# allenai/OLMoASR

Hardware: AMD Instinct MI355X
Metric: audio-seconds/sec/node (train step) (higher is better)
Workload: dtype bf16

## Files before the change

include/oasr_testing.h:

```cpp
#ifndef OASR_TESTING_H
#define OASR_TESTING_H
#include "oasr.h"
#ifdef __cplusplus
extern "C" {
#endif

int oasr_profile_gemm(int enable);
int oasr_gemm_set_variant(int v);
int oasr_decode_set_ln_fold(int mode);
int oasr_span_set_side_streams(int mode);
int oasr_span_side_streams(void);
int oasr_xcd_plan_debug(int d, int H, int Te, int M, int L, int team, int wg, int* out, int max_blocks);
int oasr_wide_supports_debug(int d, int H, int Te, int S_max, int L, int M, int nwg, int V);
int oasr_wide_plan_debug(int d, int nwg, int N, int K, int wg, int wave, int* out, int max_units);
int oasr_xcd_offsets_ok_debug(const int64_t* layer0, long long lstride, long long cache_lstride, int d, int Te, int L, int M);
int oasr_attention_set_pingpong(int on);
int oasr_attention_set_span_grid(int on);
int oasr_gemm_set_stagger(int sleeps, int phases);
int oasr_gemm_force_general(int on);
int oasr_test_gemm(const oasr_gemm_args* a, float* colsum_scratch, int atomic_on_pp, int raster_gm, int stagger, int stagger_phases, void* stream);
int oasr_profile_gemm_records(char* buf, int cap);
int oasr_gemm_route_debug(int M, int N, int K, int ta, int tb, int a_view, int b_view, int split_k, int atomic, int atomic_on_pp, int outputs,
                          int sides, long long ldc, long long ldr, long long ldu, int misalign, int colsum, int colsum_scratch, int forced_path,
                          int pp_schedule, int geom_env, char* symbol, int cap, int* post);
int oasr_profile_gemm_collect(double* ms4, double* flops4, int64_t* count4, char* by_symbol , int cap);
int oasr_probe_lds_oob(const void* src_u16 , void* dst_u16 , void* stream);
int oasr_probe_tr16(const void* src_bf16 , void* dst_bf16 , void* stream);
int oasr_test_span_tables(const int32_t* span_host, int B, int S, const int64_t* targets, int32_t* rows_out, int32_t* span_out,
                          int64_t* targets_rows_out, int64_t* active_rows_out, void* stream);
int oasr_test_span_block_tables(const int32_t* span_host, int B, int S, int H, const int64_t* targets, int32_t* rows_out, int32_t* span_out,
                                int64_t* targets_rows_out, int32_t* blk128_out, int32_t* blk256_out, int32_t* counts_out, void* stream);

int oasr_test_embedding_fwd(const int64_t* tok, const float* E, const float* pos, void* x, int dtype, int B, int S, int d, int64_t n_embed,
                            const int32_t* rows, void* stream);
int oasr_test_embedding_bwd(const int64_t* tok, const void* dx, int dtype, float* dE, float* dpos, int B, int S, int d, int64_t pad_id,
                            int64_t n_embed, const int32_t* rows, const int32_t* span, void* stream);
int oasr_test_colsum(const void* x, int dtype, int64_t ld, int64_t M, int ncols, float* out, void* stream);
int oasr_test_conv2_col2im_dgelu(const void* dA, const void* u1, void* dpre1, int dtype, int B, int T1, int d, void* stream);
int oasr_test_conv1_col2im_mel(const void* dcol, int dtype, float* dmel, int B, int T1, int n_mels, void* stream);
int oasr_test_mel_to_time_major(const float* mel, void* out, int dtype, int B, int n_mels, int T, const float* clip_max, void* stream);
int oasr_test_pack_conv_weight(const float* w, void* dst, int dtype, int co, int ci, int ldk, void* stream);
int oasr_test_unpack_conv_grad(const float* g, float* dw, int co, int ci, int ldk, void* stream);
int oasr_test_pack_embedding(const float* e, void* dst, int rows, int rows_pad, int d, void* stream);
int oasr_test_dgelu_mul(const void* dy, const void* u, void* out, int dtype, int64_t n, void* stream);
int oasr_test_dlogits_from_f32(const float* src, int V, int64_t rows, int64_t ld, void* dst, int dtype, void* stream);
int oasr_test_logits_to_f32(const void* logits, int dtype, int64_t ld, int64_t rows, int V, float* out, void* stream);
int oasr_test_layernorm_bwd(const void* dy, const void* x, const float* gamma, const float* mean, const float* rstd, const void* dres, void* dx,
                            float* dgamma, float* dbeta, float* dsum, int dtype, int64_t rows, int d, void* stream);

int oasr_test_dtw_host(const float* cost, int64_t ld, int N, int M, int negate, int32_t* text_indices, int32_t* time_indices, int32_t* path_len,
                       void* workspace);

int oasr_test_argmax_rows(const void* logits, int dtype, int64_t ld, int V, int64_t n_rows, const int32_t* rows, const int32_t* span, int B, int S,
                          int32_t* pred_out, void* stream);

int oasr_test_cross_entropy(void* logits, int dtype, int64_t ld, int V, const int64_t* targets, int64_t rows, int64_t ignore, float gscale,
                            int32_t* n_valid_dev, float* row_loss, float* loss_out, int write_grad, float label_smoothing, float z_loss,
                            float* row_parts, void* stream);

#ifdef __cplusplus
}
#endif
#endif
```

olmoasr_amd/_native.py:

```python
import ctypes as C
import os

import torch

_HERE = os.path.dirname(os.path.abspath(__file__))
LIB_PATH = os.environ.get("OASR_LIB") or os.path.join(_HERE, "liboasr.so")
_lib = None


class NativeError(RuntimeError):
    pass


class Dims(C.Structure):
    _fields_ = [(n, C.c_int) for n in ("n_mels", "n_audio_ctx", "n_audio_state", "n_audio_head", "n_audio_layer",
                                       "n_vocab", "n_text_ctx", "n_text_state", "n_text_head", "n_text_layer")]


class Operand(C.Structure):
    _fields_ = [("ptr", C.c_void_p), ("ld", C.c_int64), ("rpb", C.c_int), ("bstride", C.c_int64), ("lead", C.c_int),
                ("kvalid", C.c_int), ("trail_from", C.c_int)]


class GemmArgs(C.Structure):
    _fields_ = [("A", Operand), ("B", Operand), ("M", C.c_int), ("N", C.c_int), ("K", C.c_int), ("ta", C.c_int),
                ("tb", C.c_int), ("alpha", C.c_float), ("bias", C.c_void_p), ("act", C.c_int), ("pos", C.c_void_p),
                ("pos_period", C.c_int), ("dgelu_u", C.c_void_p), ("ldu", C.c_int64), ("resid", C.c_void_p),
                ("ldr", C.c_int64), ("out", C.c_void_p), ("out_pre", C.c_void_p), ("ldc", C.c_int64),
                ("out_f32", C.c_void_p), ("ldc32", C.c_int64), ("beta", C.c_float), ("colsum", C.c_void_p), ("atomic", C.c_int),
                ("split_k", C.c_int), ("dgelu_deriv", C.c_int)]


class AttnArgs(C.Structure):
    _fields_ = [("q", C.c_void_p), ("k", C.c_void_p), ("v", C.c_void_p), ("ldq", C.c_int64), ("ldk", C.c_int64),
                ("ldv", C.c_int64), ("bsq", C.c_int64), ("bsk", C.c_int64), ("bsv", C.c_int64), ("o", C.c_void_p),
                ("ldo", C.c_int64), ("bso", C.c_int64), ("lse", C.c_void_p), ("o_lo", C.c_void_p), ("kv_len", C.c_void_p), ("B", C.c_int),
                ("H", C.c_int), ("Tq", C.c_int), ("Tk", C.c_int), ("causal", C.c_int), ("d_o", C.c_void_p),
                ("delta", C.c_void_p), ("dq", C.c_void_p), ("dk", C.c_void_p), ("dv", C.c_void_p), ("dq_colsum", C.c_void_p),
                ("dv_colsum", C.c_void_p), ("colsum_scratch", C.c_void_p), ("qtile_flags", C.c_void_p),
                ("q_rows", C.c_void_p), ("k_rows", C.c_void_p), ("q_span", C.c_void_p),
                ("qblk128", C.c_void_p), ("qblk256", C.c_void_p), ("n128", C.c_int), ("n256", C.c_int)]


class AlignArgs(C.Structure):
    MAX_LAYERS = 32
    _fields_ = [("qk", C.c_void_p * 32), ("head_mask", C.c_uint32 * 32), ("n_layers", C.c_int32), ("H", C.c_int32), ("n_tok", C.c_int32),
                ("Tk", C.c_int32), ("n_frames", C.c_int32), ("medfilt_width", C.c_int32), ("qk_scale", C.c_float), ("reserved", C.c_int32),
                ("out", C.c_void_p), ("ldo", C.c_int64)]


class SpecAug(C.Structure):
    MAX_MASKS = 8
    _fields_ = [("freq_masks", C.c_int32), ("freq_width", C.c_int32), ("time_masks", C.c_int32), ("time_width", C.c_int32), ("fill", C.c_float)]


class EditArgs(C.Structure):
    MAX_LEN = 1023
    _fields_ = [("hyp", C.c_void_p), ("ref", C.c_void_p), ("hyp_len", C.c_void_p), ("ref_len", C.c_void_p), ("out", C.c_void_p),
                ("ld_hyp", C.c_int64), ("ld_ref", C.c_int64), ("B", C.c_int32), ("Lh", C.c_int32), ("Lr", C.c_int32), ("reserved", C.c_int32)]


class ScoreArgs(C.Structure):
    _fields_ = [(n, C.c_void_p) for n in ("mel", "xa", "tokens", "targets", "text_len", "span", "row_nll", "pred", "nll_sum", "nll_max", "n_tok",
                                          "n_hit")] + [("B", C.c_int32), ("S", C.c_int32)]


class BeamArgs(C.Structure):
    MAX_BEAM = 15
    NOT_FULL = 0x7fffffff
    _fields_ = [(n, C.c_void_p) for n in ("top_logprob", "top_token", "tokens_in", "tokens_out", "sums", "sources", "last_token", "pool_tokens",
                                          "pool_len", "pool_score", "pool_count", "pool_full_len", "short_step")] + \
               [(n, C.c_int32) for n in ("n_audio", "beam", "max_candidates", "n_ctx", "len", "reserved")] + [("eot", C.c_int64)]


class Speed(C.Structure):
    MAX_FACTORS = 8
    _fields_ = [("n_factors", C.c_int32), ("P", C.c_int32 * 8), ("Q", C.c_int32 * 8)]


class SpeedArgs(C.Structure):
    MAX_N = 1 << 26
    _fields_ = [("pcm_in", C.c_void_p), ("pcm_out", C.c_void_p), ("n_valid", C.c_void_p), ("n_out", C.c_void_p), ("factor_out", C.c_void_p),
                ("tokens_a", C.c_void_p), ("tokens_b", C.c_void_p), ("ld_in", C.c_int64), ("ld_out", C.c_int64), ("ld_tokens_a", C.c_int64),
                ("ld_tokens_b", C.c_int64), ("seed", C.c_uint64), ("first_clip", C.c_uint64), ("B", C.c_int32), ("N", C.c_int32),
                ("S", C.c_int32), ("ts_begin", C.c_int32), ("ts_max", C.c_int32), ("policy", Speed)]


class Noise(C.Structure):
    NONE = -128
    SNR_MIN, SNR_MAX = -10, 50
    _fields_ = [("prob_q16", C.c_int32), ("snr_lo_db", C.c_int32), ("snr_hi_db", C.c_int32)]


class NoiseArgs(C.Structure):
    MAX_N, MAX_ROWS = 1 << 26, 65535
    _fields_ = [("pcm_in", C.c_void_p), ("pcm_out", C.c_void_p), ("n_valid", C.c_void_p), ("bank", C.c_void_p), ("row_out", C.c_void_p),
                ("snr_out", C.c_void_p), ("gain_out", C.c_void_p), ("workspace", C.c_void_p), ("workspace_bytes", C.c_size_t),
                ("ld_in", C.c_int64), ("ld_out", C.c_int64), ("ld_bank", C.c_int64), ("seed", C.c_uint64), ("first_clip", C.c_uint64),
                ("B", C.c_int32), ("N", C.c_int32), ("M", C.c_int32), ("L", C.c_int32), ("policy", Noise), ("reserved", C.c_int32)]


class Reverb(C.Structure):
    _fields_ = [("prob_q16", C.c_int32)]


class ReverbArgs(C.Structure):
    MAX_N, MAX_ROWS, MAX_K, TAP_MAX = 1 << 26, 65535, 8192, 32639
    _fields_ = [("pcm_in", C.c_void_p), ("pcm_out", C.c_void_p), ("n_valid", C.c_void_p), ("rir", C.c_void_p), ("delay", C.c_void_p),
                ("row_out", C.c_void_p), ("workspace", C.c_void_p), ("workspace_bytes", C.c_size_t), ("ld_in", C.c_int64), ("ld_out", C.c_int64),
                ("ld_rir", C.c_int64), ("seed", C.c_uint64), ("first_clip", C.c_uint64), ("B", C.c_int32), ("N", C.c_int32), ("R", C.c_int32),
                ("K", C.c_int32), ("policy", Reverb), ("reserved", C.c_int32)]


class Telephone(C.Structure):
    MAX_CODECS = 8
    LINEAR, MULAW, ALAW = 0, 1, 2
    BP_TAPS, UP_TAPS = 129, 32
    _fields_ = [("prob_q16", C.c_int32), ("n_codecs", C.c_int32), ("codecs", C.c_int32 * 8), ("bandpass", C.c_int32)]


class TelephoneArgs(C.Structure):
    MAX_N, MAX_ROWS = 1 << 26, 65535
    _fields_ = [("pcm_in", C.c_void_p), ("pcm_out", C.c_void_p), ("n_valid", C.c_void_p), ("codec_out", C.c_void_p), ("ld_in", C.c_int64),
                ("ld_out", C.c_int64), ("seed", C.c_uint64), ("first_clip", C.c_uint64), ("B", C.c_int32), ("N", C.c_int32),
                ("policy", Telephone), ("reserved", C.c_int32)]


class TrainStepArgs(C.Structure):
    _fields_ = [(n, C.c_void_p) for n in ("mel", "xa", "tokens", "targets", "text_len", "span_host", "mel_clip_max", "loss_out", "logits_out",
                                          "pred_out", "seg_events")] + \
               [(n, C.c_int32) for n in ("B", "S", "span_forward", "accumulate_loss")] + [("loss_scale", C.c_float), ("inv_accum", C.c_float)] + \
               [("label_smoothing", C.c_float), ("z_loss", C.c_float), ("loss_parts_out", C.c_void_p), ("loss_parts_rows", C.c_void_p)]


DTW_MAX_N, DTW_MAX_M = 448, 1500
STRUCT_SIZES = [
    ("oasr_sizeof_attn_args", AttnArgs),
    ("oasr_sizeof_align_args", AlignArgs),
    ("oasr_sizeof_specaug", SpecAug),
    ("oasr_sizeof_edit_args", EditArgs),
    ("oasr_sizeof_beam_args", BeamArgs),
    ("oasr_sizeof_speed", Speed),
    ("oasr_sizeof_speed_args", SpeedArgs),
    ("oasr_sizeof_noise", Noise),
    ("oasr_sizeof_noise_args", NoiseArgs),
    ("oasr_sizeof_reverb", Reverb),
    ("oasr_sizeof_reverb_args", ReverbArgs),
    ("oasr_sizeof_telephone", Telephone),
    ("oasr_sizeof_telephone_args", TelephoneArgs),
    ("oasr_sizeof_train_step_args", TrainStepArgs),
    ("oasr_sizeof_score_args", ScoreArgs),
]
ABI_VERSION = 216
KV_TAIL_BYTES = 327680
KV_TEAM_COUNTER, KV_ERROR, KV_TEAM_EPOCH, KV_XCC_MASK, KV_WIDE_EPOCH, KV_CTRL_WORDS = 0, 1, 2, 3, 4, 5
KV_REPLICAS, KV_FLAG_STRIDE, KV_FLAGS_WORD = 8, 1024, 1024
MODE_INFER, MODE_TRAIN, MODE_TRAIN_ENC, MODE_TRAIN_DEC = 0, 1, 2, 3
ROWTAB = 16
LORA_MAX_RANK = 64


def _declare(lib):
    vp, i32, i64, f32, sz = C.c_void_p, C.c_int, C.c_int64, C.c_float, C.c_size_t
    sig = {
        "oasr_last_error": (C.c_char_p, []),
        "oasr_version": (i32, []),
        "oasr_log_mel_workspace_bytes": (sz, [i32]),
        "oasr_log_mel": (i32, [vp, i32, i32, i32, vp, vp, vp]),
        "oasr_mel_filterbank": (i32, [vp]),
        "oasr_create": (vp, [C.POINTER(Dims)]),
        "oasr_create_ex": (vp, [C.POINTER(Dims), i32]),
        "oasr_create_ex2": (vp, [C.POINTER(Dims), i32, i32]),
        "oasr_compute_dtype": (i32, [vp]),
        "oasr_create_ex3": (vp, [C.POINTER(Dims), i32, i32, vp, i32, i32, f32]),
        "oasr_lora_count": (i32, [vp]),
        "oasr_lora_merge": (i32, [vp, vp]),
        "oasr_lora_merge_op": (i32, [vp, vp, vp, i32, i32, i32, f32, i32, vp, vp]),
        "oasr_lora_grad_scratch_bytes": (sz, [i32, i32, i32]),
        "oasr_lora_grad_op": (i32, [vp, vp, vp, i32, i32, i32, f32, vp, vp, vp, vp]),
        "oasr_encode": (i32, [vp, vp, i32, vp, vp, sz, vp]),
        "oasr_kv_cache_bytes": (sz, [vp, i32]),
        "oasr_decode_step_workspace_bytes": (sz, [vp, i32]),
        "oasr_decode_begin": (i32, [vp, vp, i32, vp, vp]),
        "oasr_decode_step": (i32, [vp, vp, i32, i32, vp, vp, vp, sz, vp]),
        "oasr_decode_check": (i32, [vp, i32, vp, vp]),
        "oasr_decode_logits": (i32, [vp, vp, vp, vp, i32, i32, i32, vp, vp, sz, vp]),
        "oasr_destroy": (None, [vp]),
        "oasr_param_count": (i32, [vp]),
        "oasr_param_info": (i32, [vp, i32, C.c_char_p, i32, C.POINTER(i64), C.POINTER(i64), C.POINTER(i32), C.POINTER(i64)]),
        "oasr_param_numel": (i64, [vp]),
        "oasr_segment_count": (i32, [vp]),
        "oasr_segment_info": (i32, [vp, i32, C.POINTER(i64), C.POINTER(i64)]),
        "oasr_bind": (i32, [vp, vp, vp, vp, vp, vp]),
        "oasr_shadow_bytes": (sz, [vp]),
        "oasr_bind_shadow": (i32, [vp, vp]),
        "oasr_refresh_shadow": (i32, [vp, vp]),
        "oasr_workspace_bytes": (sz, [vp, i32, i32, i32]),
        "oasr_forward": (i32, [vp, vp, vp, vp, i32, i32, vp, vp, vp, sz, vp]),
        "oasr_sizeof_train_step_args": (sz, []),
        "oasr_train_step": (i32, [vp, C.POINTER(TrainStepArgs), vp, sz, vp]),
        "oasr_log_mel_raw": (i32, [vp, i32, i32, i32, vp, vp, vp, vp]),
        "oasr_sizeof_attn_args": (sz, []),
        "oasr_test_span_tables": (i32, [vp, i32, i32, vp, vp, vp, vp, vp, vp]),
        "oasr_test_span_block_tables": (i32, [vp, i32, i32, i32, vp, vp, vp, vp, vp, vp, vp, vp]),
        "oasr_test_embedding_fwd": (i32, [vp, vp, vp, vp, i32, i32, i32, i32, i64, vp, vp]),
        "oasr_test_embedding_bwd": (i32, [vp, vp, i32, vp, vp, i32, i32, i32, i64, i64, vp, vp, vp]),
        "oasr_test_colsum": (i32, [vp, i32, i64, i64, i32, vp, vp]),
        "oasr_test_conv2_col2im_dgelu": (i32, [vp, vp, vp, i32, i32, i32, i32, vp]),
        "oasr_test_conv1_col2im_mel": (i32, [vp, i32, vp, i32, i32, i32, vp]),
        "oasr_test_mel_to_time_major": (i32, [vp, vp, i32, i32, i32, i32, vp, vp]),
        "oasr_test_pack_conv_weight": (i32, [vp, vp, i32, i32, i32, i32, vp]),
        "oasr_test_unpack_conv_grad": (i32, [vp, vp, i32, i32, i32, vp]),
        "oasr_test_pack_embedding": (i32, [vp, vp, i32, i32, i32, vp]),
        "oasr_test_dgelu_mul": (i32, [vp, vp, vp, i32, i64, vp]),
        "oasr_test_dlogits_from_f32": (i32, [vp, i32, i64, i64, vp, i32, vp]),
        "oasr_test_logits_to_f32": (i32, [vp, i32, i64, i64, i32, vp, vp]),
        "oasr_test_layernorm_bwd": (i32, [vp, vp, vp, vp, vp, vp, vp, vp, vp, vp, i32, i64, i32, vp]),
        "oasr_train_fwd": (i32, [vp, vp, vp, vp, i32, i32, vp, vp, sz, vp]),
        "oasr_train_bwd": (i32, [vp, vp, vp, vp, i32, i32, vp, vp, sz, vp]),
        "oasr_zero_grad": (i32, [vp, vp]),
        "oasr_train_encode": (i32, [vp, vp, i32, vp, vp, sz, vp]),
        "oasr_train_encode_bwd": (i32, [vp, vp, i32, vp, vp, sz, vp]),
        "oasr_train_decode": (i32, [vp, vp, vp, vp, i32, i32, vp, vp, sz, vp]),
        "oasr_train_decode_bwd": (i32, [vp, vp, vp, vp, i32, i32, vp, vp, sz, vp]),
        "oasr_set_trainable": (i32, [vp, vp, i32]),
        "oasr_optim_step": (i32, [vp, f32, f32, f32, f32, f32, f32, f32, i64, vp, vp, vp]),
        "oasr_grad_sumsq_range": (i32, [vp, i64, i64, vp, vp, vp]),
        "oasr_optim_step_range": (i32, [vp, i64, i64, vp, vp, vp, f32, f32, f32, f32, f32, f32, f32, i64, vp]),
        "oasr_gemm": (i32, [C.POINTER(GemmArgs), vp]),
        "oasr_test_gemm": (i32, [C.POINTER(GemmArgs), vp, i32, i32, i32, i32, vp]),
        "oasr_profile_gemm_records": (i32, [C.c_char_p, i32]),
        "oasr_gemm_route_debug": (i32, [i32] * 11 + [i32, C.c_longlong, C.c_longlong, C.c_longlong] + [i32] * 6 + [C.c_char_p, i32, C.POINTER(i32)]),
        "oasr_layernorm_fwd": (i32, [vp, vp, vp, vp, vp, vp, i64, i32, vp]),
        "oasr_layernorm_bwd": (i32, [vp, vp, vp, vp, vp, vp, vp, vp, vp, i64, i32, vp]),
        "oasr_attention_fwd": (i32, [C.POINTER(AttnArgs), vp]),
        "oasr_attention_bwd": (i32, [C.POINTER(AttnArgs), vp]),
        "oasr_attention_scores": (i32, [C.POINTER(AttnArgs), i32, vp, vp]),
        "oasr_sizeof_align_args": (sz, []),
        "oasr_alignment_workspace_bytes": (sz, [i32, i32, i32]),
        "oasr_alignment_matrix": (i32, [C.POINTER(AlignArgs), vp, sz, vp]),
        "oasr_dtw_workspace_bytes": (sz, [i32, i32]),
        "oasr_dtw": (i32, [vp, i64, i32, i32, i32, vp, vp, vp, vp, sz, vp]),
        "oasr_test_dtw_host": (i32, [vp, i64, i32, i32, i32, vp, vp, vp, vp]),
        "oasr_sizeof_specaug": (sz, []),
        "oasr_spec_augment": (i32, [vp, i32, i32, i32, C.POINTER(SpecAug), C.c_uint64, C.c_uint64, vp]),
        "oasr_spec_augment_plan": (i32, [C.POINTER(SpecAug), C.c_uint64, C.c_uint64, i32, i32, vp, vp]),
        "oasr_sizeof_edit_args": (sz, []),
        "oasr_edit_counts": (i32, [C.POINTER(EditArgs), vp]),
        "oasr_edit_counts_host": (i32, [C.POINTER(EditArgs)]),
        "oasr_sizeof_score_args": (sz, []),
        "oasr_score": (i32, [vp, C.POINTER(ScoreArgs), vp, sz, vp]),
        "oasr_score_rows": (i32, [vp, i32, i64, i32, vp, vp, i32, i32, i64, vp, vp, vp]),
        "oasr_score_reduce": (i32, [vp, vp, vp, vp, i32, i32, i32, i64, vp, vp, vp, vp, vp]),
        "oasr_score_reduce_host": (i32, [vp, vp, vp, vp, i32, i32, i32, i64, vp, vp, vp, vp]),
        "oasr_sizeof_beam_args": (sz, []),
        "oasr_beam_update": (i32, [C.POINTER(BeamArgs), vp]),
        "oasr_beam_update_host": (i32, [C.POINTER(BeamArgs)]),
        "oasr_decode_reorder": (i32, [vp, vp, i32, i32, i32, vp, vp, vp]),
        "oasr_decode_reorder_host": (i32, [vp, i64, i32, i32, i32, i32, i32, i32, i32, vp]),
        "oasr_sizeof_speed": (sz, []),
        "oasr_sizeof_speed_args": (sz, []),
        "oasr_speed_perturb": (i32, [C.POINTER(SpeedArgs), vp]),
        "oasr_speed_perturb_host": (i32, [C.POINTER(SpeedArgs)]),
        "oasr_speed_plan": (i32, [C.POINTER(Speed), C.c_uint64, C.c_uint64, i32, i32, C.POINTER(i32), C.POINTER(i32), C.POINTER(i32), C.POINTER(i32)]),
        "oasr_speed_table": (i32, [i32, i32, vp, C.POINTER(i32)]),
        "oasr_sizeof_noise": (sz, []),
        "oasr_sizeof_noise_args": (sz, []),
        "oasr_noise_workspace_bytes": (sz, [i32, i32]),
        "oasr_noise_mix": (i32, [C.POINTER(NoiseArgs), vp]),
        "oasr_noise_mix_host": (i32, [C.POINTER(NoiseArgs)]),
        "oasr_noise_plan": (i32, [C.POINTER(Noise), C.c_uint64, C.c_uint64, i32, i32, C.POINTER(i32), C.POINTER(i32), C.POINTER(i32), C.POINTER(i32)]),
        "oasr_sizeof_reverb": (sz, []),
        "oasr_sizeof_reverb_args": (sz, []),
        "oasr_reverb_workspace_bytes": (sz, [i32, i32]),
        "oasr_reverb": (i32, [C.POINTER(ReverbArgs), vp]),
        "oasr_reverb_host": (i32, [C.POINTER(ReverbArgs)]),
        "oasr_reverb_plan": (i32, [C.POINTER(Reverb), C.c_uint64, C.c_uint64, i32, C.POINTER(i32), C.POINTER(i32)]),
        "oasr_sizeof_telephone": (sz, []),
        "oasr_sizeof_telephone_args": (sz, []),
        "oasr_telephone": (i32, [C.POINTER(TelephoneArgs), vp]),
        "oasr_telephone_host": (i32, [C.POINTER(TelephoneArgs)]),
        "oasr_telephone_plan": (i32, [C.POINTER(Telephone), C.c_uint64, C.c_uint64, C.POINTER(i32), C.POINTER(i32)]),
        "oasr_telephone_tables": (i32, [vp, vp]),
        "oasr_telephone_quantize_host": (i32, [vp, vp, i64, i32]),
        "oasr_test_argmax_rows": (i32, [vp, i32, i64, i32, i64, vp, vp, i32, i32, vp, vp]),
        "oasr_cross_entropy": (i32, [vp, i64, i32, vp, i64, i64, f32, vp, vp, vp, i32, vp]),
        "oasr_cross_entropy_ex": (i32, [vp, i64, i32, vp, i64, i64, f32, vp, vp, vp, i32, f32, f32, vp, vp]),
        "oasr_test_cross_entropy": (i32, [vp, i32, i64, i32, vp, i64, i64, f32, vp, vp, vp, i32, f32, f32, vp, vp]),
        "oasr_cast_f32_bf16": (i32, [vp, vp, i64, vp]),
        "oasr_pick_tokens": (i32, [vp, i64, i32, i64, vp, vp, vp, vp, vp]),
        "oasr_pick_tokens_ts": (i32, [vp, i64, i32, i64, vp, vp, vp, i64, i32, i32, i32, i32, i32, vp, vp, vp]),
        "oasr_topk_tokens": (i32, [vp, i64, i32, i64, vp, vp, vp, i64, i32, i32, i32, i32, i32, i32, vp, vp, vp]),
        "oasr_sample_tokens": (i32, [vp, i64, i32, i64, vp, vp, vp, i64, i32, i32, i32, i32, i32, f32, vp, vp, vp, vp]),
        "oasr_probe_tr16": (i32, [vp, vp, vp]),
        "oasr_probe_lds_oob": (i32, [vp, vp, vp]),
        "oasr_profile_gemm": (i32, [i32]),
        "oasr_gemm_force_general": (i32, [i32]),
        "oasr_gemm_set_stagger": (i32, [i32, i32]),
        "oasr_gemm_set_variant": (i32, [i32]),
        "oasr_decode_set_ln_fold": (i32, [i32]),
        "oasr_span_set_side_streams": (i32, [i32]),
        "oasr_span_side_streams": (i32, []),
        "oasr_xcd_plan_debug": (i32, [i32, i32, i32, i32, i32, i32, i32, vp, i32]),
        "oasr_xcd_offsets_ok_debug": (i32, [vp, C.c_longlong, C.c_longlong, i32, i32, i32, i32]),
        "oasr_wide_supports_debug": (i32, [i32, i32, i32, i32, i32, i32, i32, i32]),
        "oasr_wide_plan_debug": (i32, [i32, i32, i32, i32, i32, i32, vp, i32]),
        "oasr_attention_set_pingpong": (i32, [i32]),
        "oasr_attention_set_span_grid": (i32, [i32]),
        "oasr_profile_gemm_collect": (i32, [vp, vp, vp, C.c_char_p, i32]),
    }
    for name, (res, args) in sig.items():
        fn = getattr(lib, name)
        fn.restype = res
        fn.argtypes = args
    return list(sig)


EXPORTS = None


def _check_struct_size(handle, entry, struct):
    size = getattr(handle, entry, lambda: None)()
    if size != C.sizeof(struct):
        raise NativeError(f"{LIB_PATH}: {entry} answers {size} bytes, this binding's {struct.__name__} has {C.sizeof(struct)} "
                          "-- rebuild (__graft_entry__.build())")


def lib():
    global _lib, EXPORTS
    if _lib is None:
        if not os.path.isfile(LIB_PATH):
            raise NativeError(f"{LIB_PATH} not found: run `python -c 'import __graft_entry__ as g; g.build()'` "
                              "(hipcc --offload-arch=gfx950).  There is no CPU/PyTorch fallback for this path.")
        try:
            _lib = C.CDLL(LIB_PATH)
        except OSError as e:
            raise NativeError(f"cannot load {LIB_PATH}: {e}") from e
        handle, _lib = _lib, None
        ver = getattr(handle, "oasr_version", lambda: None)()
        if ver != ABI_VERSION:
            raise NativeError(f"{LIB_PATH}: ABI version {ver}, this binding is written for version {ABI_VERSION} -- rebuild (__graft_entry__.build())")
        _check_struct_size(handle, *STRUCT_SIZES[0])
        try:
            exports = _declare(handle)
        except AttributeError as e:
            raise NativeError(f"{LIB_PATH} (ABI {ver}) lacks an entry point this binding declares: {e} -- rebuild (__graft_entry__.build())") from e
        for row in STRUCT_SIZES[1:]:
            _check_struct_size(handle, *row)
        _lib, EXPORTS = handle, exports
    return _lib


def enable_testing_hooks():
    os.environ["OASR_TESTING_HOOKS"] = "1"


ERETRY = -4


def check(rc, what=""):
    if rc != 0:
        msg = lib().oasr_last_error()
        raise NativeError(f"{what} failed (rc={rc}): {msg.decode() if msg else ''}")


def ptr(t):
    if t is None:
        return None
    return C.c_void_p(t.data_ptr())


def stream_ptr(device=None):
    return C.c_void_p(torch.cuda.current_stream(device).cuda_stream)


STREAM = object()
_Tensor = torch.Tensor


def call(name, *args, device=None):
    fn = getattr(_lib or lib(), name)
    argv, stream_at = [], -1
    for a in args:
        if isinstance(a, _Tensor):
            if a.is_cuda:
                if device is None:
                    device = a.device
                elif a.device != device:
                    raise NativeError(f"{name}: arguments on {device} and on {a.device} -- one call, one device (nothing was launched)")
            a = a.data_ptr()
        elif a is STREAM:
            stream_at = len(argv)
        argv.append(a)
    if device is None:
        if stream_at >= 0:
            raise NativeError(f"{name}: a stream was asked for, but no argument names a device")
        rc = fn(*argv)
    else:
        with torch.cuda.device(device):
            if stream_at >= 0:
                argv[stream_at] = torch.cuda.current_stream().cuda_stream
            rc = fn(*argv)
    if rc != 0:
        check(rc, name)


def require_gpu(t, name="tensor"):
    if not (isinstance(t, torch.Tensor) and t.is_cuda):
        raise NativeError(f"{name} must be a CUDA/HIP tensor: the MI355X-native path has no CPU fallback")
```

olmoasr_amd/csrc/api.hip:

```cpp
#include <stdarg.h>

#include "../../include/oasr.h"
#include "kernels.h"

static thread_local char g_err[512] = "";

void oasr_set_error(const char* fmt, ...) {
  va_list ap;
  va_start(ap, fmt);
  vsnprintf(g_err, sizeof(g_err), fmt, ap);
  va_end(ap);
}

extern "C" const char* oasr_last_error(void) { return g_err; }
extern "C" int oasr_version(void) { return OASR_ABI_VERSION; }
extern "C" size_t oasr_sizeof_attn_args(void) { return sizeof(oasr_attn_args); }

static OperandView to_view(const oasr_operand& o) {
  return OperandView{(const bf16_t*)o.ptr, (long)o.ld, o.rpb, (long)o.bstride, o.lead, o.kvalid, o.trail_from};
}

static int to_gemm(const oasr_gemm_args* a, GemmArgs& g) {
  OASR_REQUIRE(a, "oasr_gemm: null args");
  g = gemm_defaults();
  g.A = to_view(a->A);
  g.B = to_view(a->B);
  g.M = a->M;
  g.N = a->N;
  g.K = a->K;
  g.ta = a->ta;
  g.tb = a->tb;
  g.alpha = a->alpha;
  g.bias = a->bias;
  g.act = a->act;
  g.pos = a->pos;
  g.pos_period = a->pos_period;
  g.dgelu_u = (const bf16_t*)a->dgelu_u;
  g.ldu = a->ldu;
  g.resid = (const bf16_t*)a->resid;
  g.ldr = a->ldr;
  g.out = (bf16_t*)a->out;
  g.out_pre = (bf16_t*)a->out_pre;
  g.ldc = a->ldc;
  g.out_f32 = a->out_f32;
  g.ldc32 = a->ldc32;
  g.beta = a->beta;
  g.colsum = a->colsum;
  g.atomic = a->atomic;
  g.split_k = a->split_k < 1 ? 1 : a->split_k;
  g.dgelu_deriv = a->dgelu_deriv;
  OASR_REQUIRE(a->act >= 0 && a->act <= 2, "oasr_gemm: act must be 0 (none), 1 (GELU) or 2 (GELU, out_pre = GELU')");
  return OASR_OK;
}

extern "C" int oasr_gemm(const oasr_gemm_args* a, void* stream) {
  GemmArgs g;
  const int rc = to_gemm(a, g);
  return rc ? rc : launch_gemm(g, (hipStream_t)stream);
}

extern "C" int oasr_test_gemm(const oasr_gemm_args* a, float* colsum_scratch, int atomic_on_pp, int raster_gm, int stagger, int stagger_phases,
                              void* stream) {
  GemmArgs g;
  const int rc = to_gemm(a, g);
  if (rc) return rc;
  g.colsum_scratch = colsum_scratch;
  g.atomic_on_pp = atomic_on_pp;
  g.raster_gm = raster_gm;
  g.stagger = stagger;
  g.stagger_phases = stagger_phases;
  return launch_gemm(g, (hipStream_t)stream);
}

extern "C" int oasr_profile_gemm(int enable) {
  gemm_profile_enable(enable);
  return OASR_OK;
}
extern "C" int oasr_gemm_set_variant(int v) {
  OASR_HOOK_GATE("oasr_gemm_set_variant");
  return gemm_set_variant(v);
}
extern "C" int oasr_gemm_set_stagger(int sleeps, int phases) {
  OASR_HOOK_GATE("oasr_gemm_set_stagger");
  gemm_set_stagger(sleeps, phases);
  return OASR_OK;
}
extern "C" int oasr_attention_set_pingpong(int on) {
  OASR_HOOK_GATE("oasr_attention_set_pingpong");
  attention_set_pingpong(on);
  return OASR_OK;
}
extern "C" int oasr_attention_set_span_grid(int on) {
  OASR_HOOK_GATE("oasr_attention_set_span_grid");
  attention_set_span_grid(on);
  return OASR_OK;
}
extern "C" int oasr_gemm_force_general(int on) {
  OASR_HOOK_GATE("oasr_gemm_force_general");
  gemm_force_general(on);
  return OASR_OK;
}
extern "C" int oasr_profile_gemm_records(char* buf, int cap) {
  const int n = gemm_profile_records(buf, cap);
  OASR_REQUIRE(n >= 0, "oasr_profile_gemm_records: %d bytes do not hold the launch records", cap);
  return n;
}
extern "C" int oasr_profile_gemm_collect(double* ms4, double* flops4, int64_t* count4, char* by_symbol, int cap) {
  OASR_REQUIRE(ms4 && flops4 && count4, "profile_collect: null");
  long c[4];
  int rc = gemm_profile_collect(ms4, flops4, c, by_symbol, cap);
  for (int i = 0; i < 4; ++i) count4[i] = c[i];
  return rc;
}

extern "C" int oasr_layernorm_fwd(const void* x, const float* gamma, const float* beta, void* y, float* mean, float* rstd, int64_t rows,
                                  int d, void* stream) {
  return launch_layernorm_fwd((const bf16_t*)x, gamma, beta, (bf16_t*)y, mean, rstd, rows, d, (hipStream_t)stream);
}
extern "C" int oasr_layernorm_bwd(const void* dy, const void* x, const float* gamma, const float* mean, const float* rstd,
                                  const void* dres, void* dx, float* dgamma, float* dbeta, int64_t rows, int d, void* stream) {
  return launch_layernorm_bwd((const bf16_t*)dy, (const bf16_t*)x, gamma, mean, rstd, (const bf16_t*)dres, (bf16_t*)dx, dgamma, dbeta,
                              nullptr, rows, d, (hipStream_t)stream);
}

static AttnArgs to_attn(const oasr_attn_args* a) {
  AttnArgs r;
  memset(&r, 0, sizeof(r));
  r.q = (const bf16_t*)a->q;
  r.k = (const bf16_t*)a->k;
  r.v = (const bf16_t*)a->v;
  r.ldq = a->ldq;
  r.ldk = a->ldk;
  r.ldv = a->ldv;
  r.bsq = a->bsq;
  r.bsk = a->bsk;
  r.bsv = a->bsv;
  r.o = (bf16_t*)a->o;
  r.ldo = a->ldo;
  r.bso = a->bso;
  r.lse = a->lse;
  r.o_lo = (bf16_t*)a->o_lo;
  r.kv_len = a->kv_len;
  r.B = a->B;
  r.H = a->H;
  r.Tq = a->Tq;
  r.Tk = a->Tk;
  r.causal = a->causal;
  r.d_o = (const bf16_t*)a->d_o;
  r.delta = a->delta;
  r.dq = (bf16_t*)a->dq;
  r.dk = (bf16_t*)a->dk;
  r.dv = (bf16_t*)a->dv;
  r.dq_colsum = a->dq_colsum;
  r.dv_colsum = a->dv_colsum;
  r.colsum_scratch = a->colsum_scratch;
  r.qtile_flags = a->qtile_flags;
  r.q_rows = a->q_rows;
  r.k_rows = a->k_rows;
  r.q_span = a->q_span;
  r.qblk128 = a->qblk128;
  r.qblk256 = a->qblk256;
  r.n128 = a->n128;
  r.n256 = a->n256;
  return r;
}
extern "C" int oasr_attention_fwd(const oasr_attn_args* a, void* stream) {
  OASR_REQUIRE(a, "oasr_attention_fwd: null args");
  return launch_attention_fwd(to_attn(a), (hipStream_t)stream);
}
extern "C" int oasr_attention_bwd(const oasr_attn_args* a, void* stream) {
  OASR_REQUIRE(a, "oasr_attention_bwd: null args");
  return launch_attention_bwd(to_attn(a), (hipStream_t)stream);
}
extern "C" int oasr_attention_scores(const oasr_attn_args* a, int dtype, float* scores, void* stream) {
  OASR_REQUIRE(a && scores, "oasr_attention_scores: null args");
  OASR_REQUIRE(dtype == OASR_DTYPE_BF16 || dtype == OASR_DTYPE_F32, "oasr_attention_scores: dtype %d (0 = bf16 operands, 1 = fp32 operands)", dtype);
  if (dtype == OASR_DTYPE_BF16) return launch_attention_scores(to_attn(a), scores, (hipStream_t)stream);
  AttnArgsF f;
  memset(&f, 0, sizeof(f));
  f.q = (const float*)a->q, f.k = (const float*)a->k;
  f.ldq = a->ldq, f.ldk = a->ldk, f.bsq = a->bsq, f.bsk = a->bsk;
  f.kv_len = a->kv_len;
  f.B = a->B, f.H = a->H, f.Tq = a->Tq, f.Tk = a->Tk, f.causal = a->causal;
  f.q_rows = a->q_rows, f.k_rows = a->k_rows;
  return launch_attention_scores(f, scores, (hipStream_t)stream);
}

extern "C" size_t oasr_sizeof_align_args(void) { return sizeof(oasr_align_args); }
extern "C" int oasr_alignment_matrix(const oasr_align_args* a, void* workspace, size_t workspace_bytes, void* stream) {
  return launch_alignment_matrix(a, workspace, workspace_bytes, (hipStream_t)stream);
}
extern "C" int oasr_dtw(const float* cost, int64_t ld, int N, int M, int negate, int32_t* text_indices, int32_t* time_indices, int32_t* path_len,
                        void* workspace, size_t workspace_bytes, void* stream) {
  return launch_dtw(cost, (long)ld, N, M, negate, text_indices, time_indices, path_len, workspace, workspace_bytes, (hipStream_t)stream);
}

extern "C" size_t oasr_sizeof_specaug(void) { return sizeof(oasr_specaug); }
extern "C" int oasr_spec_augment(float* mel, int B, int n_mels, int T, const oasr_specaug* policy, uint64_t seed, uint64_t first_clip,
                                 void* stream) {
  return launch_spec_augment(mel, B, n_mels, T, policy, seed, first_clip, (hipStream_t)stream);
}

extern "C" int oasr_edit_counts(const oasr_edit_args* a, void* stream) { return launch_edit_counts(a, (hipStream_t)stream); }

extern "C" int oasr_score_rows(const void* logits, int dtype, int64_t ld, int V, const int64_t* targets, const int32_t* span, int B, int S,
                               int64_t ignore, float* row_nll, int32_t* pred, void* stream) {
  OASR_REQUIRE(dtype == OASR_DTYPE_BF16 || dtype == OASR_DTYPE_F32, "oasr_score_rows: dtype %d (0 = bf16, 1 = fp32 logits)", dtype);
  if (dtype == OASR_DTYPE_BF16)
    return launch_score_rows((const bf16_t*)logits, (long)ld, V, targets, span, B, S, (long)ignore, row_nll, pred, (hipStream_t)stream);
  return launch_score_rows((const float*)logits, (long)ld, V, targets, span, B, S, (long)ignore, row_nll, pred, (hipStream_t)stream);
}
extern "C" int oasr_score_reduce(const float* row_nll, const int32_t* pred, const int64_t* targets, const int32_t* span, int B, int S, int V,
                                 int64_t ignore, float* nll_sum, float* nll_max, int32_t* n_tok, int32_t* n_hit, void* stream) {
  return launch_score_reduce(row_nll, pred, targets, span, B, S, V, (long)ignore, nll_sum, nll_max, n_tok, n_hit, (hipStream_t)stream);
}

extern "C" int oasr_beam_update(const oasr_beam_args* a, void* stream) { return launch_beam_update(a, (hipStream_t)stream); }

extern "C" size_t oasr_sizeof_speed(void) { return sizeof(oasr_speed); }
extern "C" size_t oasr_sizeof_speed_args(void) { return sizeof(oasr_speed_args); }
extern "C" int oasr_speed_perturb(const oasr_speed_args* a, void* stream) { return launch_speed_perturb(a, (hipStream_t)stream); }

extern "C" size_t oasr_sizeof_noise(void) { return sizeof(oasr_noise); }
extern "C" size_t oasr_sizeof_noise_args(void) { return sizeof(oasr_noise_args); }
extern "C" size_t oasr_noise_workspace_bytes(int B, int N) { return (B < 1 || N < 1) ? 0 : noise_workspace_bytes(B, N); }
extern "C" int oasr_noise_mix(const oasr_noise_args* a, void* stream) { return launch_noise_mix(a, (hipStream_t)stream); }

extern "C" size_t oasr_sizeof_reverb(void) { return sizeof(struct oasr_reverb); }
extern "C" size_t oasr_sizeof_reverb_args(void) { return sizeof(oasr_reverb_args); }
extern "C" size_t oasr_reverb_workspace_bytes(int R, int K) {
  return (R < 1 || R > 65535 || K < 1 || K > 8192) ? 0 : reverb_workspace_bytes(R, K);
}
extern "C" int oasr_reverb(const oasr_reverb_args* a, void* stream) { return launch_reverb(a, (hipStream_t)stream); }

extern "C" size_t oasr_sizeof_telephone(void) { return sizeof(struct oasr_telephone); }
extern "C" size_t oasr_sizeof_telephone_args(void) { return sizeof(oasr_telephone_args); }
extern "C" int oasr_telephone(const oasr_telephone_args* a, void* stream) { return launch_telephone(a, (hipStream_t)stream); }

extern "C" int oasr_test_span_tables(const int32_t* span_host, int B, int S, const int64_t* targets, int32_t* rows_out, int32_t* span_out,
                                     int64_t* targets_rows_out, int64_t* active_rows_out, void* stream) {
  OASR_REQUIRE(active_rows_out, "oasr_test_span_tables: null");
  long act = 0;
  const int rc = launch_build_span_tables(span_host, B, S, targets, 51864, rows_out, span_out, targets_rows_out, &act, (hipStream_t)stream);
  *active_rows_out = act;
  return rc;
}

extern "C" int oasr_test_span_block_tables(const int32_t* span_host, int B, int S, int H, const int64_t* targets, int32_t* rows_out,
                                           int32_t* span_out, int64_t* targets_rows_out, int32_t* blk128_out, int32_t* blk256_out,
                                           int32_t* counts_out, void* stream) {
  OASR_REQUIRE(counts_out, "oasr_test_span_block_tables: null");
  long act = 0;
  SpanBlockTables blk{H, blk128_out, blk256_out, 0, 0};
  const int rc = launch_build_span_tables(span_host, B, S, targets, 51864, rows_out, span_out, targets_rows_out, &act, (hipStream_t)stream, &blk);
  counts_out[0] = blk.n128;
  counts_out[1] = blk.n256;
  return rc;
}

#define OASR_TEST_DTYPE(name) \
  OASR_REQUIRE(dtype == OASR_DTYPE_BF16 || dtype == OASR_DTYPE_F32, name ": dtype %d (0 = bf16, 1 = fp32 activations)", dtype)

extern "C" int oasr_test_embedding_fwd(const int64_t* tok, const float* E, const float* pos, void* x, int dtype, int B, int S, int d,
                                       int64_t n_embed, const int32_t* rows, void* stream) {
  OASR_TEST_DTYPE("oasr_test_embedding_fwd");
  if (dtype == OASR_DTYPE_BF16) return launch_embedding_fwd(tok, E, pos, (bf16_t*)x, B, S, d, (long)n_embed, (hipStream_t)stream, rows);
  return launch_embedding_fwd(tok, E, pos, (float*)x, B, S, d, (long)n_embed, (hipStream_t)stream, rows);
}
extern "C" int oasr_test_embedding_bwd(const int64_t* tok, const void* dx, int dtype, float* dE, float* dpos, int B, int S, int d, int64_t pad_id,
                                       int64_t n_embed, const int32_t* rows, const int32_t* span, void* stream) {
  OASR_TEST_DTYPE("oasr_test_embedding_bwd");
  OASR_REQUIRE(!span || rows, "oasr_test_embedding_bwd: span comes with a chunk-row table");
  if (dtype == OASR_DTYPE_BF16)
    return launch_embedding_bwd(tok, (const bf16_t*)dx, dE, dpos, B, S, d, (long)pad_id, (long)n_embed, (hipStream_t)stream, rows, span);
  return launch_embedding_bwd(tok, (const float*)dx, dE, dpos, B, S, d, (long)pad_id, (long)n_embed, (hipStream_t)stream, rows, span);
}
extern "C" int oasr_test_colsum(const void* x, int dtype, int64_t ld, int64_t M, int ncols, float* out, void* stream) {
  OASR_TEST_DTYPE("oasr_test_colsum");
  if (dtype == OASR_DTYPE_BF16) return launch_colsum_accum((const bf16_t*)x, (long)ld, (long)M, ncols, out, (hipStream_t)stream);
  return launch_colsum_accum((const float*)x, (long)ld, (long)M, ncols, out, (hipStream_t)stream);
}
extern "C" int oasr_test_conv2_col2im_dgelu(const void* dA, const void* u1, void* dpre1, int dtype, int B, int T1, int d, void* stream) {
  OASR_TEST_DTYPE("oasr_test_conv2_col2im_dgelu");
  OASR_REQUIRE(B > 0 && T1 > 0 && d > 0, "oasr_test_conv2_col2im_dgelu: bad shape (B=%d T1=%d d=%d)", B, T1, d);
  if (dtype == OASR_DTYPE_BF16) return launch_conv2_col2im_dgelu((const bf16_t*)dA, (const bf16_t*)u1, (bf16_t*)dpre1, B, T1, d, (hipStream_t)stream);
  return launch_conv2_col2im_dgelu((const float*)dA, (const float*)u1, (float*)dpre1, B, T1, d, (hipStream_t)stream);
}
extern "C" int oasr_test_conv1_col2im_mel(const void* dcol, int dtype, float* dmel, int B, int T1, int n_mels, void* stream) {
  OASR_TEST_DTYPE("oasr_test_conv1_col2im_mel");
  if (dtype == OASR_DTYPE_BF16) return launch_conv1_col2im_mel((const bf16_t*)dcol, dmel, B, T1, n_mels, (hipStream_t)stream);
  return launch_conv1_col2im_mel((const float*)dcol, dmel, B, T1, n_mels, (hipStream_t)stream);
}
extern "C" int oasr_test_mel_to_time_major(const float* mel, void* out, int dtype, int B, int n_mels, int T, const float* clip_max, void* stream) {
  OASR_TEST_DTYPE("oasr_test_mel_to_time_major");
  OASR_REQUIRE(B > 0 && n_mels > 0 && T > 0, "oasr_test_mel_to_time_major: bad shape (B=%d n_mels=%d T=%d)", B, n_mels, T);
  if (dtype == OASR_DTYPE_BF16) return launch_mel_to_time_major(mel, (bf16_t*)out, B, n_mels, T, (hipStream_t)stream, clip_max);
  return launch_mel_to_time_major(mel, (float*)out, B, n_mels, T, (hipStream_t)stream, clip_max);
}
extern "C" int oasr_test_pack_conv_weight(const float* w, void* dst, int dtype, int co, int ci, int ldk, void* stream) {
  OASR_TEST_DTYPE("oasr_test_pack_conv_weight");
  OASR_REQUIRE(co > 0 && ci > 0, "oasr_test_pack_conv_weight: bad shape (co=%d ci=%d)", co, ci);
  if (dtype == OASR_DTYPE_BF16) return launch_pack_conv_weight(w, (bf16_t*)dst, co, ci, ldk, (hipStream_t)stream);
  return launch_pack_conv_weight(w, (float*)dst, co, ci, ldk, (hipStream_t)stream);
}
extern "C" int oasr_test_unpack_conv_grad(const float* g, float* dw, int co, int ci, int ldk, void* stream) {
  OASR_REQUIRE(co > 0 && ci > 0, "oasr_test_unpack_conv_grad: bad shape (co=%d ci=%d)", co, ci);
  return launch_unpack_conv_grad(g, dw, co, ci, ldk, (hipStream_t)stream);
}
extern "C" int oasr_test_pack_embedding(const float* e, void* dst, int rows, int rows_pad, int d, void* stream) {
  OASR_REQUIRE(rows > 0 && d > 0, "oasr_test_pack_embedding: bad shape (rows=%d d=%d)", rows, d);
  return launch_pack_embedding(e, (bf16_t*)dst, rows, rows_pad, d, (hipStream_t)stream);
}
extern "C" int oasr_test_dgelu_mul(const void* dy, const void* u, void* out, int dtype, int64_t n, void* stream) {
  OASR_TEST_DTYPE("oasr_test_dgelu_mul");
  OASR_REQUIRE(n > 0, "oasr_test_dgelu_mul: n = %lld", (long long)n);
  if (dtype == OASR_DTYPE_BF16) return launch_dgelu_mul((const bf16_t*)dy, (const bf16_t*)u, (bf16_t*)out, (long)n, (hipStream_t)stream);
  return launch_dgelu_mul((const float*)dy, (const float*)u, (float*)out, (long)n, (hipStream_t)stream);
}
extern "C" int oasr_test_dlogits_from_f32(const float* src, int V, int64_t rows, int64_t ld, void* dst, int dtype, void* stream) {
  OASR_TEST_DTYPE("oasr_test_dlogits_from_f32");
  OASR_REQUIRE(rows > 0 && V > 0, "oasr_test_dlogits_from_f32: bad shape");
  if (dtype == OASR_DTYPE_BF16) return launch_dlogits_from_f32(src, V, (long)rows, (long)ld, (bf16_t*)dst, (hipStream_t)stream);
  return launch_dlogits_from_f32(src, V, (long)rows, (long)ld, (float*)dst, (hipStream_t)stream);
}
extern "C" int oasr_test_logits_to_f32(const void* logits, int dtype, int64_t ld, int64_t rows, int V, float* out, void* stream) {
  OASR_TEST_DTYPE("oasr_test_logits_to_f32");
  OASR_REQUIRE(logits && out && rows > 0 && V > 0 && V <= ld, "oasr_test_logits_to_f32: bad args");
  if (dtype == OASR_DTYPE_BF16) return launch_logits_to_f32((const bf16_t*)logits, (long)ld, (long)rows, V, out, (hipStream_t)stream);
  return launch_logits_to_f32((const float*)logits, (long)ld, (long)rows, V, out, (hipStream_t)stream);
}
extern "C" int oasr_test_layernorm_bwd(const void* dy, const void* x, const float* gamma, const float* mean, const float* rstd, const void* dres,
                                       void* dx, float* dgamma, float* dbeta, float* dsum, int dtype, int64_t rows, int d, void* stream) {
  OASR_TEST_DTYPE("oasr_test_layernorm_bwd");
  if (dtype == OASR_DTYPE_BF16)
    return launch_layernorm_bwd((const bf16_t*)dy, (const bf16_t*)x, gamma, mean, rstd, (const bf16_t*)dres, (bf16_t*)dx, dgamma, dbeta, dsum,
                                (long)rows, d, (hipStream_t)stream);
  return launch_layernorm_bwd((const float*)dy, (const float*)x, gamma, mean, rstd, (const float*)dres, (float*)dx, dgamma, dbeta, dsum, (long)rows, d,
                              (hipStream_t)stream);
}

extern "C" int oasr_test_argmax_rows(const void* logits, int dtype, int64_t ld, int V, int64_t n_rows, const int32_t* rows, const int32_t* span, int B,
                                     int S, int32_t* pred_out, void* stream) {
  OASR_TEST_DTYPE("oasr_test_argmax_rows");
  if (dtype == OASR_DTYPE_BF16)
    return launch_argmax_rows((const bf16_t*)logits, (long)ld, V, (long)n_rows, rows, span, B, S, pred_out, (hipStream_t)stream);
  return launch_argmax_rows((const float*)logits, (long)ld, V, (long)n_rows, rows, span, B, S, pred_out, (hipStream_t)stream);
}

template <typename T>
static int cross_entropy_chain(const char* who, T* logits, int64_t ld, int V, const int64_t* targets, int64_t rows, int64_t ignore, float gscale,
                               int32_t* n_valid_dev, float* row_loss, float* loss_out, int write_grad, float label_smoothing, float z_loss,
                               float* row_parts, hipStream_t st) {
  int rc = check_ce_reg(who, label_smoothing, z_loss);
  if (rc) return rc;
  CeReg reg;
  reg.eps = label_smoothing;
  reg.z = z_loss;
  reg.parts = row_parts;
  reg.parts_stride = (long)rows;
  rc = launch_count_valid(targets, rows, ignore, V, n_valid_dev, st);
  if (rc) return rc;
  rc = launch_cross_entropy(logits, ld, V, targets, rows, ignore, gscale, n_valid_dev, row_loss, write_grad, st, reg);
  if (rc) return rc;
  if (loss_out) rc = launch_loss_reduce(row_loss, rows, n_valid_dev, 1.0f, loss_out, 0, st);
  return rc;
}
extern "C" int oasr_cross_entropy_ex(void* logits, int64_t ld, int V, const int64_t* targets, int64_t rows, int64_t ignore, float gscale,
                                     int32_t* n_valid_dev, float* row_loss, float* loss_out, int write_grad, float label_smoothing, float z_loss,
                                     float* row_parts, void* stream) {
  return cross_entropy_chain("oasr_cross_entropy_ex", (bf16_t*)logits, ld, V, targets, rows, ignore, gscale, n_valid_dev, row_loss, loss_out,
                             write_grad, label_smoothing, z_loss, row_parts, (hipStream_t)stream);
}
extern "C" int oasr_test_cross_entropy(void* logits, int dtype, int64_t ld, int V, const int64_t* targets, int64_t rows, int64_t ignore, float gscale,
                                       int32_t* n_valid_dev, float* row_loss, float* loss_out, int write_grad, float label_smoothing,
                                       float z_loss, float* row_parts, void* stream) {
  OASR_TEST_DTYPE("oasr_test_cross_entropy");
  if (dtype == OASR_DTYPE_BF16)
    return cross_entropy_chain("oasr_test_cross_entropy", (bf16_t*)logits, ld, V, targets, rows, ignore, gscale, n_valid_dev, row_loss, loss_out,
                               write_grad, label_smoothing, z_loss, row_parts, (hipStream_t)stream);
  return cross_entropy_chain("oasr_test_cross_entropy", (float*)logits, ld, V, targets, rows, ignore, gscale, n_valid_dev, row_loss, loss_out,
                             write_grad, label_smoothing, z_loss, row_parts, (hipStream_t)stream);
}
extern "C" int oasr_cross_entropy(void* logits, int64_t ld, int V, const int64_t* targets, int64_t rows, int64_t ignore, float gscale,
                                  int32_t* n_valid_dev, float* row_loss, float* loss_out, int write_grad, void* stream) {
  return oasr_cross_entropy_ex(logits, ld, V, targets, rows, ignore, gscale, n_valid_dev, row_loss, loss_out, write_grad, 0.f, 0.f, nullptr, stream);
}

extern "C" int oasr_pick_tokens(const float* logits, int64_t ld, int V, int64_t rows, const float* mask, const float* mask2, int64_t* tok,
                                float* logprob, void* stream) {
  SelectArgs a{logits, ld, V, rows, mask, mask2};
  a.tok = tok;
  a.logprob = logprob;
  return launch_pick_tokens(a, (hipStream_t)stream);
}
extern "C" int oasr_pick_tokens_ts(const float* logits, int64_t ld, int V, int64_t rows, const float* mask, const float* mask2,
                                   const int64_t* history, int64_t history_ld, int n_history, int timestamp_begin, int eot, int no_timestamps,
                                   int max_initial_index, int64_t* tok, float* logprob, void* stream) {
  return launch_pick_tokens_ts({logits, ld, V, rows, mask, mask2, history, history_ld, n_history, timestamp_begin, eot, no_timestamps,
                                max_initial_index, tok, logprob}, (hipStream_t)stream);
}
extern "C" int oasr_topk_tokens(const float* logits, int64_t ld, int V, int64_t rows, const float* mask, const float* mask2,
                                const int64_t* history, int64_t history_ld, int n_history, int timestamp_begin, int eot, int no_timestamps,
                                int max_initial_index, int K, int64_t* tok, float* logprob, void* stream) {
  return launch_topk_tokens_ts({logits, ld, V, rows, mask, mask2, history, history_ld, n_history, timestamp_begin, eot, no_timestamps,
                                max_initial_index, tok, logprob}, K, (hipStream_t)stream);
}
extern "C" int oasr_sample_tokens(const float* logits, int64_t ld, int V, int64_t rows, const float* mask, const float* mask2,
                                  const int64_t* history, int64_t history_ld, int n_history, int timestamp_begin, int eot, int no_timestamps,
                                  int max_initial_index, float temperature, const float* uniforms, int64_t* tok, float* logprob, void* stream) {
  return launch_sample_tokens_ts({logits, ld, V, rows, mask, mask2, history, history_ld, n_history, timestamp_begin, eot, no_timestamps,
                                  max_initial_index, tok, logprob}, temperature, uniforms, (hipStream_t)stream);
}

extern "C" int oasr_cast_f32_bf16(const float* src, void* dst, int64_t n, void* stream) {
  return launch_cast_f32_bf16(src, (bf16_t*)dst, n, (hipStream_t)stream);
}

typedef __attribute__((address_space(3))) s16x4_t* lds_s16x4_ptr_t;
__global__ void probe_tr16_kernel(const bf16_t* __restrict__ src, bf16_t* __restrict__ dst) {
  __shared__ __attribute__((aligned(16))) bf16_t tile[16 * 64];
  const int l = threadIdx.x;
  for (int i = l; i < 16 * 64; i += 64) tile[i] = src[i];
  __syncthreads();
  const int row = (l >> 4) * 4 + ((l & 15) >> 2), col = ((l & 15) & 3) * 4;
  const s16x4_t v = __builtin_amdgcn_ds_read_tr16_b64_v4i16((lds_s16x4_ptr_t)(tile + row * 64 + col));
  for (int j = 0; j < 4; ++j) dst[l * 4 + j] = (bf16_t)v[j];
}
typedef __attribute__((address_space(3))) void* lds_void_ptr_t;
__global__ void probe_lds_oob_kernel(const bf16_t* __restrict__ src, bf16_t* __restrict__ dst) {
  __shared__ __attribute__((aligned(16))) bf16_t tile[64 * 8];
  const int l = threadIdx.x;
  for (int i = l; i < 64 * 8; i += 64) tile[i] = 0xAAAA;
  __syncthreads();
  const __amdgpu_buffer_rsrc_t rs = __builtin_amdgcn_make_buffer_rsrc(const_cast<bf16_t*>(src), 0, 64 * 16, 0x00020000);
  const unsigned off = l < 32 ? l * 16 : 0x80000000u;
  __builtin_amdgcn_raw_ptr_buffer_load_lds(rs, (lds_void_ptr_t)tile, 16, off, 0, 0, 0);
  __syncthreads();
  for (int i = l; i < 64 * 8; i += 64) dst[i] = tile[i];
}
extern "C" int oasr_probe_lds_oob(const void* src, void* dst, void* stream) {
  hipLaunchKernelGGL(probe_lds_oob_kernel, dim3(1), dim3(64), 0, (hipStream_t)stream, (const bf16_t*)src, (bf16_t*)dst);
  OASR_LAUNCH_CHECK();
  return OASR_OK;
}
extern "C" int oasr_probe_tr16(const void* src, void* dst, void* stream) {
  hipLaunchKernelGGL(probe_tr16_kernel, dim3(1), dim3(64), 0, (hipStream_t)stream, (const bf16_t*)src, (bf16_t*)dst);
  OASR_LAUNCH_CHECK();
  return OASR_OK;
}
```

olmoasr_amd/csrc/attention.hip:

```cpp
#include "attention_common.h"

namespace {

int g_attn_pingpong = 1;
int g_attn_span_grid = 1;

bool span_grid(const AttnArgs& a) { return g_attn_span_grid && a.q_rows && a.q_span && a.qblk128 && a.qblk256; }

int check_args(const AttnArgs& a, bool bwd) {
  OASR_REQUIRE(a.q && a.k && a.v && a.o, "attention: null pointer");
  OASR_REQUIRE(a.B > 0 && a.H > 0 && a.Tq > 0 && a.Tk > 0, "attention: bad shape");
  OASR_REQUIRE((a.ldq % 8) == 0 && (a.ldk % 8) == 0 && (a.ldv % 8) == 0 && (a.ldo % 8) == 0, "attention: strides must be multiples of 8");
  OASR_REQUIRE(!a.causal || a.Tq == a.Tk, "attention: causal needs Tq == Tk");
  if (bwd) OASR_REQUIRE(a.d_o && a.lse && a.delta && a.dq && a.dk && a.dv, "attention_bwd: null pointer");
  if (bwd) OASR_REQUIRE((!a.dq_colsum && !a.dv_colsum) || a.colsum_scratch, "attention_bwd: fused bias gradients need colsum_scratch");
  OASR_REQUIRE(!a.k_rows || a.q_rows, "attention: k_rows needs q_rows");
  OASR_REQUIRE(!a.q_span || a.q_rows, "attention: q_span needs q_rows");
  OASR_REQUIRE(!a.q_rows || ((a.Tq % 64) == 0 && a.Tq <= 64 * OASR_ROWTAB), "attention: chunked query rows need Tq %% 64 == 0 and Tq <= %d", 64 * OASR_ROWTAB);
  OASR_REQUIRE(!a.k_rows || ((a.Tk % 64) == 0 && a.Tk <= 64 * OASR_ROWTAB), "attention: chunked key rows need Tk %% 64 == 0 and Tk <= %d", 64 * OASR_ROWTAB);
  OASR_REQUIRE(!a.qblk128 == !a.qblk256, "attention: the 128- and the 256-query block tables come together");
  OASR_REQUIRE(!a.qblk128 || (a.n128 >= 0 && a.n128 <= a.B * cdiv(a.Tq, 128) && a.n256 >= 0 && a.n256 <= a.B * cdiv(a.Tq, 256) && a.n256 <= a.n128 &&
                              a.n128 <= 2 * a.n256),
               "attention: block counts n128 = %d, n256 = %d do not fit B = %d, Tq = %d", a.n128, a.n256, a.B, a.Tq);
  return OASR_OK;
}

}

void attention_set_pingpong(int on) { g_attn_pingpong = on; }
void attention_set_span_grid(int on) { g_attn_span_grid = on; }

int launch_attention_fwd(const AttnArgs& a, hipStream_t s) {
  int rc = check_args(a, false);
  if (rc) return rc;
  if (a.Tq == 1 && a.Tk <= 1536 && !a.o_lo && !a.q_rows) {
    attn_launch_decode(a, s);
    OASR_LAUNCH_CHECK();
    return OASR_OK;
  }
  dim3 grid(cdiv(a.Tq, 128) * a.B * a.H);
  AttnArgs r = a;
  if (span_grid(a)) {
    if (a.n128 == 0) return OASR_OK;
    grid = dim3(a.n128 * a.H);
  } else {
    r.qblk128 = r.qblk256 = nullptr;
  }
  attn_launch_fwd(r, grid, s);
  OASR_LAUNCH_CHECK();
  return OASR_OK;
}

int launch_attention_bwd(const AttnArgs& a, hipStream_t s) {
  int rc = check_args(a, true);
  if (rc) return rc;
  dim3 gq(cdiv(a.Tq, 128) * a.B * a.H), gk(cdiv(a.Tk, 128) * a.B * a.H), gq256(cdiv(a.Tq, 256) * a.B * a.H);
  const bool rows = a.q_rows != nullptr;
  const int d = a.H * 64;
  const long rq = (long)a.B * cdiv(a.Tq, 128), rk = (long)a.B * cdiv(a.Tk, 128);
  AttnArgs aq = a, ak = a;
  const bool cq = rows && span_grid(a), ck = cq && a.k_rows != nullptr && a.Tk == a.Tq;
  if (!cq) aq.qblk128 = aq.qblk256 = nullptr;
  if (!ck) ak.qblk128 = ak.qblk256 = nullptr;
  if (cq) {
    if (a.n128 == 0) return OASR_OK;
    gq = dim3(a.n128 * a.H);
    gq256 = dim3(a.n256 * a.H);
    if (ck) gk = gq;
    const long zrows = (a.dq_colsum ? rq : 0) + (ck && a.dv_colsum ? rk : 0);
    float* z0 = a.dq_colsum ? a.colsum_scratch : a.colsum_scratch + rq * d;
    if (zrows) OASR_CHECK_HIP(hipMemsetAsync(z0, 0, (size_t)zrows * d * sizeof(float), s));
  }
  const bool pp = !a.causal && !a.kv_len && g_attn_pingpong && (!rows || (!a.k_rows && a.Tq <= 512));
  if (pp) {
    attn_launch_bwd_dq_pp(aq, gq256, s);
    rc = attn_launch_bwd_dkdv_pp(a, dim3(cdiv(a.Tk, 256) * a.B * a.H), s);
    if (rc) return rc;
  } else {
    attn_launch_bwd_dq(aq, gq, s);
    attn_launch_bwd_dkdv(ak, gk, s);
  }
  OASR_LAUNCH_CHECK();
  if (a.dq_colsum) {
    int rc2 = launch_colsum_accum(a.colsum_scratch, d, rq, d, a.dq_colsum, s);
    if (rc2) return rc2;
  }
  if (a.dv_colsum) {
    int rc2 = launch_colsum_accum(a.colsum_scratch + rq * d, d, rk, d, a.dv_colsum, s);
    if (rc2) return rc2;
  }
  return OASR_OK;
}
```

olmoasr_amd/csrc/attention_bwd_dkdv.hip:

```cpp
#include "attention_common.h"

namespace {

__device__ __forceinline__ int wave_max_i(int v) {
#pragma unroll
  for (int o = 32; o > 0; o >>= 1) {
    const int t = __shfl_xor(v, o, 64);
    v = t > v ? t : v;
  }
  return v;
}

__device__ __forceinline__ int last_nonzero_qtile(const int32_t* flags, int n, int lane) {
  int last = -1;
  for (int i = lane; i < n; i += 64)
    if (flags[i] != 0) last = i;
  return __builtin_amdgcn_readfirstlane(wave_max_i(last));
}

template <bool CAUSAL, bool ROWS>
__global__ __launch_bounds__(256, 2) void attn_bwd_dkdv_kernel(AttnArgs a) {
  constexpr int STAGE = 2 * TILE + 512;
  __shared__ __attribute__((aligned(16))) char smem[2 * STAGE];
  const int tid = threadIdx.x, lane = tid & 63, wave = tid >> 6, hh = lane >> 5;
  const int nkb = (a.Tk + 127) >> 7;
  const int bid = xcd_remap(blockIdx.x, gridDim.x);
  const BlockId id = block_id<ROWS>(a.qblk128, bid, nkb, a.H);
  const int b = id.b, h = id.h, kblk = id.blk;
  const int k0 = kblk * 128;
  const int mykey = k0 + wave * 32 + (lane & 31);
  const bool krows = ROWS && a.k_rows != nullptr;
  const int q_lim = (ROWS && a.q_span) ? min(a.q_span[b], a.Tq) : a.Tq;
  const long dv_scratch_off0 = (long)a.B * ((a.Tq + 127) >> 7) * a.H * 64;
  if (krows && a.q_span && k0 >= q_lim) {
    if (a.dv_colsum && tid < 64) a.colsum_scratch[dv_scratch_off0 + ((long)(b * nkb + kblk) * a.H + h) * 64 + tid] = 0.f;
    return;
  }
  const bool w_store = !(krows && a.q_span) || k0 + wave * 32 < q_lim;
  const int mykey_c = !w_store ? k0 + (lane & 31) : (mykey < a.Tk ? mykey : a.Tk - 1);

  const int kv_len = clamped_kv_len(a, b);

  const bf16_t* kp = row_at(a.k, krows, a.k_rows, b, mykey_c, a.ldk, a.bsk, h);
  const bf16_t* vp = row_at(a.v, krows, a.k_rows, b, mykey_c, a.ldv, a.bsv, h);
  bf16x8_t kf[4], vf[4];
#pragma unroll
  for (int ds = 0; ds < 4; ++ds) {
    kf[ds] = ld_frag_global(kp + ds * 16 + hh * 8);
    vf[ds] = ld_frag_global(vp + ds * 16 + hh * 8);
  }
  f32x16_t dkT[2], dvT[2];
#pragma unroll
  for (int i = 0; i < 2; ++i)
#pragma unroll
    for (int r = 0; r < 16; ++r) {
      dkT[i][r] = 0.f;
      dvT[i][r] = 0.f;
    }

  const TileSrc qsrc = ROWS ? tile_src(a.q + h * 64, a.ldq, a.B * a.Tq, tid) : tile_src(a.q + (long)b * a.bsq + h * 64, a.ldq, a.Tq, tid);
  const TileSrc dosrc = ROWS ? tile_src(a.d_o + h * 64, a.ldo, a.B * a.Tq, tid) : tile_src(a.d_o + (long)b * a.bso + h * 64, a.ldo, a.Tq, tid);
  const float* lse_b = a.lse + ((long)b * a.H + h) * a.Tq;
  const float* delta_b = a.delta + ((long)b * a.H + h) * a.Tq;

  int nqt = (a.Tq + 63) >> 6;
  if (a.qtile_flags) nqt = last_nonzero_qtile(a.qtile_flags + ((long)b * a.H + h) * nqt, nqt, lane) + 1;
  if (ROWS && (q_lim >> 6) < nqt) nqt = q_lim >> 6;
  const int t_begin = (CAUSAL && k0 < kv_len) ? (k0 >> 6) : 0;
  const bool any = k0 < kv_len && t_begin < nqt;

  u32x4_t rq[2], rd[2];
  float rstat = 0.f;
  auto issue = [&](int t) {
    const int qr0 = ROWS ? __builtin_amdgcn_readfirstlane(a.q_rows[b * OASR_ROWTAB + t]) : t * 64;
    tile_issue(qsrc, qr0, rq);
    tile_issue(dosrc, qr0, rd);
    if (tid < 128) {
      int qi = t * 64 + (tid & 63);
      qi = qi < a.Tq ? qi : a.Tq - 1;
      rstat = tid < 64 ? lse_b[qi] * LOG2E : delta_b[qi];
    }
  };
  auto commit = [&](char* st) {
    tile_commit(st, tid, rq);
    tile_commit(st + TILE, tid, rd);
    if (tid < 128) ((float*)(st + 2 * TILE))[tid] = rstat;
  };
  const long dv_scratch_off = dv_scratch_off0;
  if (!any) {
    if (a.dv_colsum && tid < 64) a.colsum_scratch[dv_scratch_off + ((long)(b * nkb + kblk) * a.H + h) * 64 + tid] = 0.f;
    if (mykey < a.Tk && w_store) {
      bf16_t* dkp0 = row_at(a.dk, krows, a.k_rows, b, mykey, a.ldk, a.bsk, h);
      bf16_t* dvp0 = row_at(a.dv, krows, a.k_rows, b, mykey, a.ldv, a.bsv, h);
      const u32x4_t z = {0u, 0u, 0u, 0u};
#pragma unroll
      for (int i = 0; i < 4; ++i) {
        *(u32x4_t*)(dkp0 + hh * 32 + i * 8) = z;
        *(u32x4_t*)(dvp0 + hh * 32 + i * 8) = z;
      }
    }
    return;
  }
  issue(t_begin);
  commit(smem);
  __syncthreads();
  for (int t = t_begin; t < nqt; ++t) {
    const int cur = (t - t_begin) & 1;
    const char* st = smem + cur * STAGE;
    const char* qb = st;
    const char* dob = st + TILE;
    const float* stat = (const float*)(st + 2 * TILE);
    const bool more = t + 1 < nqt;
    if (more) issue(t + 1);
#pragma unroll
    for (int qt = 0; qt < 2; ++qt) {
      f32x16_t s, dp;
#pragma unroll
      for (int r = 0; r < 16; ++r) {
        s[r] = 0.f;
        dp[r] = 0.f;
      }
#pragma unroll
      for (int ds = 0; ds < 4; ++ds) {
        s = MFMA(frag_rows(qb, qt * 32, ds, lane), kf[ds], s);
        dp = MFMA(frag_rows(dob, qt * 32, ds, lane), vf[ds], dp);
      }
      const int key_hi = k0 + wave * 32 + 31;
      const bool full = (t * 64 + qt * 32 + 32 <= a.Tq) && (key_hi < kv_len) && (!CAUSAL || key_hi <= t * 64 + qt * 32);
      if (full) {
        const f32x2_t c2 = {SCALE * LOG2E, SCALE * LOG2E};
#pragma unroll
        for (int g4 = 0; g4 < 4; ++g4) {
          const int ql = qt * 32 + 8 * g4 + 4 * hh;
          const f32x4_t l4 = *(const f32x4_t*)(stat + ql);
          const f32x4_t d4 = *(const f32x4_t*)(stat + 64 + ql);
#pragma unroll
          for (int i = 0; i < 4; i += 2) {
            const int r = 4 * g4 + i;
            const f32x2_t s2 = {s[r], s[r + 1]}, dp2 = {dp[r], dp[r + 1]}, nl2 = {-l4[i], -l4[i + 1]}, nd2 = {-d4[i], -d4[i + 1]};
            const f32x2_t p2 = pk_exp2(pk_fma(s2, c2, nl2));
            const f32x2_t ds2 = p2 * (dp2 + nd2);
            s[r] = p2[0];
            s[r + 1] = p2[1];
            dp[r] = ds2[0];
            dp[r + 1] = ds2[1];
          }
        }
      } else {
#pragma unroll
        for (int g4 = 0; g4 < 4; ++g4) {
          const int ql = qt * 32 + 8 * g4 + 4 * hh;
          const f32x4_t l4 = *(const f32x4_t*)(stat + ql);
          const f32x4_t d4 = *(const f32x4_t*)(stat + 64 + ql);
#pragma unroll
          for (int i = 0; i < 4; ++i) {
            const int r = 4 * g4 + i;
            const int qg = t * 64 + ql + i;
            const bool ok = (qg < a.Tq) && (mykey < kv_len) && (!CAUSAL || mykey <= qg);
            const float p = ok ? __builtin_amdgcn_exp2f(fmaf(s[r], SCALE * LOG2E, -l4[i])) : 0.f;
            s[r] = p;
            dp[r] = p * (dp[r] - d4[i]);
          }
        }
      }
#pragma unroll
      for (int u = 0; u < 2; ++u) {
        const bf16x8_t pf = pack_half(s, u);
        const bf16x8_t dsf = pack_half(dp, u);
#pragma unroll
        for (int dt = 0; dt < 2; ++dt) {
          dvT[dt] = MFMA(frag_cols(dob, qt * 32 + 16 * u, dt * 32, lane), pf, dvT[dt]);
          dkT[dt] = MFMA(frag_cols(qb, qt * 32 + 16 * u, dt * 32, lane), dsf, dkT[dt]);
        }
      }
    }
    if (more) commit(smem + (cur ^ 1) * STAGE);
    __syncthreads();
  }
  {
    char* stg = smem + wave * 4096;
    const int rows_valid = w_store ? a.Tk - (k0 + wave * 32) : 0;
    const long krow0 = krows ? (long)chunk_row(a.k_rows, b, k0 + wave * 32) : 0;
    store_rows_bf16(stg, dkT, SCALE, krows ? a.dk + krow0 * a.ldk + h * 64 : a.dk + (long)b * a.bsk + (long)(k0 + wave * 32) * a.ldk + h * 64,
                    a.ldk, rows_valid, lane);
    float* wsum = (float*)(smem + 16384);
    store_rows_bf16(stg, dvT, 1.0f, krows ? a.dv + krow0 * a.ldv + h * 64 : a.dv + (long)b * a.bsv + (long)(k0 + wave * 32) * a.ldv + h * 64,
                    a.ldv, rows_valid, lane, a.dv_colsum ? wsum + wave * 64 : nullptr);
    if (a.dv_colsum) {
      __syncthreads();
      if (tid < 64)
        a.colsum_scratch[dv_scratch_off + ((long)(b * nkb + kblk) * a.H + h) * 64 + tid] =
            (wsum[tid] + wsum[64 + tid]) + (wsum[128 + tid] + wsum[192 + tid]);
    }
  }
}

constexpr int KSTAT = 2048;
constexpr int KLDS = KSTAT + PNS * PSTG;

__device__ __forceinline__ void glds4_asm(const u32x4_t rs, unsigned lds_addr, unsigned voff) {
  asm volatile("s_mov_b32 m0, %0\n\ts_nop 0\n\tbuffer_load_dword %1, %2, 0 offen lds" ::"s"(lds_addr), "v"(voff), "s"(rs) : "memory");
}

template <bool ROWS>
__global__ __launch_bounds__(512, 1) void attn_bwd_dkdv_pp_kernel(AttnArgs a) {
  extern __shared__ __attribute__((aligned(1024))) char smem[];
  const int tid = threadIdx.x, lane = tid & 63, wave = __builtin_amdgcn_readfirstlane(tid >> 6), hh = lane >> 5;
  const int grp = wave >> 2;
  const unsigned smem_a = (unsigned)(size_t)smem;
  const int nkb = (a.Tk + 255) >> 8;
  const int bid = xcd_remap(blockIdx.x, gridDim.x);
  const int bh = bid / nkb;
  const int b = bh / a.H, h = bh - b * a.H;
  const int k0 = (bid - bh * nkb) * 256;
  const int mykey = k0 + wave * 32 + (lane & 31);
  const int mykey_c = mykey < a.Tk ? mykey : a.Tk - 1;

  const bf16_t* kp = a.k + (long)b * a.bsk + (long)mykey_c * a.ldk + h * 64;
  const bf16_t* vp = a.v + (long)b * a.bsv + (long)mykey_c * a.ldv + h * 64;
  bf16x8_t kf[4], vf[4];
#pragma unroll
  for (int ds = 0; ds < 4; ++ds) {
    const u32x4_t k4 = *(const u32x4_t*)(kp + ds * 16 + hh * 8);
    const u32x4_t v4 = *(const u32x4_t*)(vp + ds * 16 + hh * 8);
    u32x4_t kn, vn;
#pragma unroll
    for (int i = 0; i < 4; ++i) {
      kn[i] = pack_bf2(bf_lo(k4[i]) * -0.125f, bf_hi(k4[i]) * -0.125f);
      vn[i] = v4[i] ^ 0x80008000u;
    }
    kf[ds] = __builtin_bit_cast(bf16x8_t, kn);
    vf[ds] = __builtin_bit_cast(bf16x8_t, vn);
  }
  asm volatile("" ::"v"(kf[3]), "v"(vf[3]));
  asm volatile("s_waitcnt vmcnt(0)" ::: "memory");

  int ntiles = (a.Tq + 63) >> 6;
  if (a.qtile_flags) ntiles = last_nonzero_qtile(a.qtile_flags + ((long)b * a.H + h) * ntiles, ntiles, lane) + 1;
  if (ROWS && a.q_span) ntiles = min(ntiles, min(a.q_span[b], a.Tq) >> 6);
  const int ngroups = (ntiles + PNS - 1) / PNS;
  const PipeSrc1 qsrc = ROWS ? pipe_src1(a.q + h * 64, a.ldq, a.B * a.Tq, wave, lane) : pipe_src1(a.q + (long)b * a.bsq + h * 64, a.ldq, a.Tq, wave, lane);
  const PipeSrc1 dosrc = ROWS ? pipe_src1(a.d_o + h * 64, a.ldo, a.B * a.Tq, wave, lane) : pipe_src1(a.d_o + (long)b * a.bso + h * 64, a.ldo, a.Tq, wave, lane);
  int qrow[8];
  if (ROWS) {
#pragma unroll
    for (int i = 0; i < 8; ++i) qrow[i] = i < ntiles ? __builtin_amdgcn_readfirstlane(a.q_rows[b * OASR_ROWTAB + i]) : 0x3fffffff;
  }
  auto qrow_of = [&](int tile) {
    int r = 0x3fffffff;
#pragma unroll
    for (int i = 0; i < 8; ++i) r = tile == i ? qrow[i] : r;
    return r;
  };
  u32x4_t srs;
  {
    const unsigned long addr = (unsigned long)(((wave & 1) ? a.delta : a.lse) + ((long)b * a.H + h) * a.Tq);
    srs[0] = (unsigned)addr;
    srs[1] = (unsigned)(addr >> 32) & 0xffffu;
    srs[2] = (unsigned)(a.Tq * 4);
    srs[3] = 0x00020000u;
  }
  auto dma_tile = [&](int tile, int stage) {
    const unsigned dst = smem_a + KSTAT + stage * PSTG + wave * 1024;
    if (ROWS) {
      const int r0 = qrow_of(tile);
      const unsigned qo = r0 == 0x3fffffff ? 0x7fffff00u : (unsigned)r0 * (unsigned)(a.ldq * 2);
      const unsigned oo = r0 == 0x3fffffff ? 0x7fffff00u : (unsigned)r0 * (unsigned)(a.ldo * 2);
      glds16_asm(qsrc.rs, dst, r0 == 0x3fffffff ? qo : qsrc.voff + qo);
      glds16_asm(dosrc.rs, dst + TILE, r0 == 0x3fffffff ? oo : dosrc.voff + oo);
      glds4_asm(srs, smem_a + stage * 512 + (wave & 1) * 256, r0 == 0x3fffffff ? 0x7fffff00u : (unsigned)(lane * 4 + tile * 256));
    } else {
      glds16_asm(qsrc.rs, dst, qsrc.voff + (unsigned)tile * qsrc.tile_bytes);
      glds16_asm(dosrc.rs, dst + TILE, dosrc.voff + (unsigned)tile * dosrc.tile_bytes);
      glds4_asm(srs, smem_a + stage * 512 + (wave & 1) * 256, (unsigned)(lane * 4 + tile * 256));
    }
  };

  int ar[4], ac[2][2];
#pragma unroll
  for (int ds = 0; ds < 4; ++ds) ar[ds] = KSTAT + tile_addr(lane & 31, ds * 2 + hh);
  {
    const int G = lane >> 4, i = lane & 15;
    const int row = 4 * (G >> 1) + (i >> 2);
#pragma unroll
    for (int dt = 0; dt < 2; ++dt) {
      const int col = dt * 32 + (G & 1) * 16 + (i & 3) * 4;
      ac[dt][0] = KSTAT + tile_addr(row, col >> 3) + (col & 7) * 2;
      ac[dt][1] = KSTAT + tile_addr(row + 8, col >> 3) + (col & 7) * 2;
    }
  }
  auto rd_rows = [&](int off, int ds) { return *(const bf16x8_t*)(smem + ar[ds] + off); };
  auto rd_tr = [&](int off, int dt, int half) {
    return __builtin_amdgcn_ds_read_tr16_b64_v4i16((lds_s16x4_ptr)(smem + ac[dt][half] + off));
  };
  const int astat = hh * 16;

  bf16x8_t Aq[4], Ado[4];
  s16x4_t cq[2][2][2], cdo[2][2][2];
  f32x16_t dkT[2], dvT[2], S[2], dP[2];
#pragma unroll
  for (int i = 0; i < 2; ++i)
#pragma unroll
    for (int r = 0; r < 16; ++r) {
      dkT[i][r] = 0.f;
      dvT[i][r] = 0.f;
    }

  auto load_seg = [&](int t, int st, int kt) {
    if (kt == 0) dma_tile(t + 3, (st + 3) & 3);
    const int a_st = kt ? ((st + 1) & 3) : st;
    const int a_off = a_st * PSTG + (kt ^ 1) * 32 * 128;
    const int c_off = st * PSTG + kt * 32 * 128;
    const int s_off = a_st * 512 + (kt ^ 1) * 128 + astat;
    const int n = kt ^ 1;
#pragma unroll
    for (int ds = 0; ds < 4; ++ds) {
      Aq[ds] = rd_rows(a_off, ds);
      Ado[ds] = rd_rows(a_off + TILE, ds);
    }
#pragma unroll
    for (int g4 = 0; g4 < 4; ++g4) {
      const f32x4_t l4 = *(const f32x4_t*)(smem + s_off + g4 * 32);
      const f32x4_t d4 = *(const f32x4_t*)(smem + s_off + 256 + g4 * 32);
#pragma unroll
      for (int i = 0; i < 4; ++i) {
        S[n][4 * g4 + i] = l4[i];
        dP[n][4 * g4 + i] = d4[i];
      }
    }
#pragma unroll
    for (int u = 0; u < 2; ++u)
#pragma unroll
      for (int dt = 0; dt < 2; ++dt)
#pragma unroll
        for (int hf = 0; hf < 2; ++hf) {
          cq[u][dt][hf] = rd_tr(c_off + u * 16 * 128, dt, hf);
          cdo[u][dt][hf] = rd_tr(c_off + TILE + u * 16 * 128, dt, hf);
        }
    if (kt == 0) asm volatile("s_waitcnt vmcnt(6)" ::: "memory");
    asm volatile("s_waitcnt lgkmcnt(0)" ::: "memory");
  };
  auto compute_seg = [&](int kt) {
    const int n = kt ^ 1;
#pragma unroll
    for (int ds = 0; ds < 4; ++ds) {
      S[n] = MFMA(Aq[ds], kf[ds], S[n]);
      dP[n] = MFMA(Ado[ds], vf[ds], dP[n]);
    }
    u32x4_t pf[2], dsf[2];
#pragma unroll
    for (int j = 0; j < 8; ++j) {
      const float p0 = __builtin_amdgcn_exp2f(S[kt][2 * j] * -LOG2E);
      const float p1 = __builtin_amdgcn_exp2f(S[kt][2 * j + 1] * -LOG2E);
      pf[j >> 2][j & 3] = pack_bf2(p0, p1);
      dsf[j >> 2][j & 3] = pack_bf2(p0 * dP[kt][2 * j], p1 * dP[kt][2 * j + 1]);
    }
#pragma unroll
    for (int u = 0; u < 2; ++u)
#pragma unroll
      for (int dt = 0; dt < 2; ++dt) {
        const s16x8_t c1 = __builtin_shufflevector(cdo[u][dt][0], cdo[u][dt][1], 0, 1, 2, 3, 4, 5, 6, 7);
        const s16x8_t c2 = __builtin_shufflevector(cq[u][dt][0], cq[u][dt][1], 0, 1, 2, 3, 4, 5, 6, 7);
        dvT[dt] = MFMA(__builtin_bit_cast(bf16x8_t, c1), __builtin_bit_cast(bf16x8_t, pf[u]), dvT[dt]);
        dkT[dt] = MFMA(__builtin_bit_cast(bf16x8_t, c2), __builtin_bit_cast(bf16x8_t, dsf[u]), dkT[dt]);
      }
#pragma unroll
    for (int i = 0; i < 8; ++i) {
      __builtin_amdgcn_sched_group_barrier(0x008, 1, 0);
      __builtin_amdgcn_sched_group_barrier(0x402, 6, 0);
    }
#pragma unroll
    for (int i = 0; i < 4; ++i) {
      __builtin_amdgcn_sched_group_barrier(0x008, 1, 0);
      __builtin_amdgcn_sched_group_barrier(0x402, 4, 0);
    }
    __builtin_amdgcn_sched_group_barrier(0x008, 4, 0);
  };

  if (ntiles > 0) {
  dma_tile(0, 0);
  dma_tile(1, 1);
  dma_tile(2, 2);
  asm volatile("s_waitcnt vmcnt(6)" ::: "memory");
  ATTN_BARRIER();
#pragma unroll
  for (int ds = 0; ds < 4; ++ds) {
    Aq[ds] = rd_rows(0, ds);
    Ado[ds] = rd_rows(TILE, ds);
  }
#pragma unroll
  for (int g4 = 0; g4 < 4; ++g4) {
    const f32x4_t l4 = *(const f32x4_t*)(smem + astat + g4 * 32);
    const f32x4_t d4 = *(const f32x4_t*)(smem + astat + 256 + g4 * 32);
#pragma unroll
    for (int i = 0; i < 4; ++i) {
      S[0][4 * g4 + i] = l4[i];
      dP[0][4 * g4 + i] = d4[i];
    }
  }
#pragma unroll
  for (int ds = 0; ds < 4; ++ds) {
    S[0] = MFMA(Aq[ds], kf[ds], S[0]);
    dP[0] = MFMA(Ado[ds], vf[ds], dP[0]);
  }
  ATTN_FENCE();
  load_seg(0, 0, 0);
  ATTN_BARRIER();
  if (grp == 1) ATTN_BARRIER();

  for (int g = 0; g < ngroups; ++g) {
#pragma unroll
    for (int st = 0; st < PNS; ++st) {
      const int t = g * PNS + st;
      compute_seg(0);
      ATTN_BARRIER();
      load_seg(t, st, 1);
      ATTN_BARRIER();
      compute_seg(1);
      ATTN_BARRIER();
      load_seg(t + 1, (st + 1) & 3, 0);
      ATTN_BARRIER();
    }
  }
  if (grp == 0) ATTN_BARRIER();
  asm volatile("s_waitcnt vmcnt(0)" ::: "memory");
  }
  __syncthreads();
  {
    char* stg = smem + wave * 4096;
    const int rows_valid = a.Tk - (k0 + wave * 32);
    store_rows_bf16(stg, dkT, -SCALE, a.dk + (long)b * a.bsk + (long)(k0 + wave * 32) * a.ldk + h * 64, a.ldk, rows_valid, lane);
    float* wsum = (float*)(smem + 32768);
    store_rows_bf16(stg, dvT, 1.0f, a.dv + (long)b * a.bsv + (long)(k0 + wave * 32) * a.ldv + h * 64, a.ldv, rows_valid, lane,
                    a.dv_colsum ? wsum + wave * 64 : nullptr);
    if (a.dv_colsum) {
      __syncthreads();
      if (tid < 128) {
        const int half = tid >> 6, c = tid & 63;
        const int nkb128 = (a.Tk + 127) >> 7;
        const int blk128 = (bid - bh * nkb) * 2 + half;
        const long dv_scratch_off = (long)a.B * ((a.Tq + 127) >> 7) * a.H * 64;
        if (blk128 < nkb128)
          a.colsum_scratch[dv_scratch_off + ((long)(b * nkb128 + blk128) * a.H + h) * 64 + c] =
              (wsum[half * 256 + c] + wsum[half * 256 + 64 + c]) + (wsum[half * 256 + 128 + c] + wsum[half * 256 + 192 + c]);
      }
    }
  }
}

}

void attn_launch_bwd_dkdv(const AttnArgs& a, dim3 grid, hipStream_t s) {
  static void (*const kern[2][2])(AttnArgs) = {{attn_bwd_dkdv_kernel<false, false>, attn_bwd_dkdv_kernel<false, true>},
                                               {attn_bwd_dkdv_kernel<true, false>, attn_bwd_dkdv_kernel<true, true>}};
  hipLaunchKernelGGL(kern[a.causal != 0][a.q_rows != nullptr], grid, dim3(256), 0, s, a);
}

int attn_launch_bwd_dkdv_pp(const AttnArgs& a, dim3 grid, hipStream_t s) {
  static void (*const kern[2])(AttnArgs) = {attn_bwd_dkdv_pp_kernel<false>, attn_bwd_dkdv_pp_kernel<true>};
  static LdsAttrOnce attr[2];
  const int rows = a.q_rows != nullptr;
  const int rc = ensure_dynamic_lds(attr[rows], (const void*)kern[rows], KLDS);
  if (rc) return rc;
  hipLaunchKernelGGL(kern[rows], grid, dim3(512), KLDS, s, a);
  return OASR_OK;
}
```

olmoasr_amd/csrc/attention_bwd_dq.hip:

```cpp
#include "attention_common.h"

namespace {

template <bool CAUSAL, bool ROWS>
__global__ __launch_bounds__(256, 2) void attn_bwd_dq_kernel(AttnArgs a) {
  __shared__ __attribute__((aligned(16))) char smem[4 * TILE];
  const int tid = threadIdx.x, lane = tid & 63, wave = tid >> 6, hh = lane >> 5;
  const int nqb = (a.Tq + 127) >> 7;
  const int bid = xcd_remap(blockIdx.x, gridDim.x);
  const BlockId id = block_id<ROWS>(a.qblk128, bid, nqb, a.H);
  const int b = id.b, h = id.h, qblk = id.blk;
  const int q0 = qblk * 128;
  const int myq = q0 + wave * 32 + (lane & 31);
  const bool krows = ROWS && a.k_rows != nullptr;
  const int q_lim = (ROWS && a.q_span) ? min(a.q_span[b], a.Tq) : a.Tq;
  if (ROWS && q0 >= q_lim) {
    if (a.dq_colsum && tid < 64) a.colsum_scratch[((long)(b * nqb + qblk) * a.H + h) * 64 + tid] = 0.f;
    return;
  }
  const bool w_act = !ROWS || q0 + wave * 32 < q_lim;
  const int myq_c = !w_act ? q0 + (lane & 31) : (myq < a.Tq ? myq : a.Tq - 1);

  bf16x8_t qf[4], dof[4];
  float delta, lse2;
  dq_row_setup<ROWS>(a, b, h, myq, myq_c, w_act, hh, qf, dof, delta, lse2);

  const int kv_len = clamped_kv_len(a, b);
  int kv_end = kv_len;
  if (CAUSAL) kv_end = kv_end < q0 + 128 ? kv_end : q0 + 128;
  int ntiles = kv_end > 0 ? (kv_end + 63) >> 6 : 1;
  if (a.qtile_flags) {
    __shared__ int nzs[4];
    bool nz = false;
#pragma unroll
    for (int ds = 0; ds < 4; ++ds) {
      const u32x4_t d4 = __builtin_bit_cast(u32x4_t, dof[ds]);
      nz = nz || ((d4[0] | d4[1] | d4[2] | d4[3]) & 0x7fff7fffu) != 0u;
    }
    const bool wnz = __any(nz);
    if (lane == 0) nzs[wave] = wnz ? 1 : 0;
    __syncthreads();
    const int t0nz = nzs[0] | nzs[1], t1nz = nzs[2] | nzs[3];
    if (tid == 0) {
      const int ntq = (a.Tq + 63) >> 6, tq = q0 >> 6;
      int32_t* f = a.qtile_flags + ((long)b * a.H + h) * ntq;
      if (tq < ntq) f[tq] = t0nz;
      if (tq + 1 < ntq) f[tq + 1] = t1nz;
    }
    if (!(t0nz | t1nz)) ntiles = 0;
  }
  const TileSrc ksrc = krows ? tile_src(a.k + h * 64, a.ldk, a.B * a.Tk, tid) : tile_src(a.k + (long)b * a.bsk + h * 64, a.ldk, a.Tk, tid);
  const TileSrc vsrc = krows ? tile_src(a.v + h * 64, a.ldv, a.B * a.Tk, tid) : tile_src(a.v + (long)b * a.bsv + h * 64, a.ldv, a.Tk, tid);
  auto krow0 = [&](int t) { return krows ? __builtin_amdgcn_readfirstlane(a.k_rows[b * OASR_ROWTAB + t]) : t * 64; };

  f32x16_t dqT[2];
#pragma unroll
  for (int i = 0; i < 2; ++i)
#pragma unroll
    for (int r = 0; r < 16; ++r) dqT[i][r] = 0.f;

  u32x4_t rk[2], rv[2];
  tile_issue(ksrc, krow0(0), rk);
  tile_issue(vsrc, krow0(0), rv);
  tile_commit(smem, tid, rk);
  tile_commit(smem + TILE, tid, rv);
  __syncthreads();
  for (int t = 0; t < ntiles; ++t) {
    const char* kb = smem + (t & 1) * 2 * TILE;
    const char* vb = kb + TILE;
    const bool more = t + 1 < ntiles;
    if (more) {
      const int r0 = krow0(t + 1);
      tile_issue(ksrc, r0, rk);
      tile_issue(vsrc, r0, rv);
    }
#pragma unroll
    for (int kt = 0; kt < 2; ++kt) {
      f32x16_t sT, dpT;
#pragma unroll
      for (int r = 0; r < 16; ++r) {
        sT[r] = 0.f;
        dpT[r] = 0.f;
      }
#pragma unroll
      for (int ds = 0; ds < 4; ++ds) {
        sT = MFMA(frag_rows(kb, kt * 32, ds, lane), qf[ds], sT);
        dpT = MFMA(frag_rows(vb, kt * 32, ds, lane), dof[ds], dpT);
      }
      const bool full = (t * 64 + kt * 32 + 32 <= kv_len) && (!CAUSAL || (t * 64 + kt * 32 + 31 <= q0 + wave * 32));
      if (full) {
        const f32x2_t c2 = {SCALE * LOG2E, SCALE * LOG2E}, nl2 = {-lse2, -lse2}, nd2 = {-delta, -delta};
#pragma unroll
        for (int r = 0; r < 16; r += 2) {
          const f32x2_t s2 = {sT[r], sT[r + 1]}, dp2 = {dpT[r], dpT[r + 1]};
          const f32x2_t ds2 = pk_exp2(pk_fma(s2, c2, nl2)) * (dp2 + nd2);
          sT[r] = ds2[0];
          sT[r + 1] = ds2[1];
        }
      } else {
#pragma unroll
        for (int r = 0; r < 16; ++r) {
          const int key = t * 64 + kt * 32 + acc_row(r, hh);
          const bool ok = (key < kv_len) && (!CAUSAL || key <= myq);
          const float p = ok ? __builtin_amdgcn_exp2f(fmaf(sT[r], SCALE * LOG2E, -lse2)) : 0.f;
          sT[r] = p * (dpT[r] - delta);
        }
      }
#pragma unroll
      for (int u = 0; u < 2; ++u) {
        const bf16x8_t dsf = pack_half(sT, u);
#pragma unroll
        for (int dt = 0; dt < 2; ++dt) dqT[dt] = MFMA(frag_cols(kb, kt * 32 + 16 * u, dt * 32, lane), dsf, dqT[dt]);
      }
    }
    if (more) {
      char* nb = smem + ((t + 1) & 1) * 2 * TILE;
      tile_commit(nb, tid, rk);
      tile_commit(nb + TILE, tid, rv);
    }
    __syncthreads();
  }
  float* wsum = (float*)(smem + 16384);
  {
    const long drow0 = row_at(0L, ROWS, a.q_rows, b, q0 + wave * 32, a.ldq, a.bsq, h);
    store_rows_bf16(smem + wave * 4096, dqT, SCALE, a.dq + drow0, a.ldq, w_act ? a.Tq - (q0 + wave * 32) : 0, lane,
                    a.dq_colsum ? wsum + wave * 64 : nullptr);
  }
  if (a.dq_colsum) {
    __syncthreads();
    if (tid < 64)
      a.colsum_scratch[((long)(b * nqb + qblk) * a.H + h) * 64 + tid] =
          (wsum[tid] + wsum[64 + tid]) + (wsum[128 + tid] + wsum[192 + tid]);
  }
}

template <bool ROWS>
__global__ __launch_bounds__(512, 1) void attn_bwd_dq_pp_kernel(AttnArgs a) {
  __shared__ __attribute__((aligned(1024))) char smem[PNS * PSTG];
  const int tid = threadIdx.x, lane = tid & 63, wave = __builtin_amdgcn_readfirstlane(tid >> 6), hh = lane >> 5;
  const int grp = wave >> 2;
  const unsigned smem_a = (unsigned)(size_t)smem;
  const int nqb = (a.Tq + 255) >> 8;
  const int bid = xcd_remap(blockIdx.x, gridDim.x);
  const BlockId id = block_id<ROWS>(a.qblk256, bid, nqb, a.H);
  const int b = id.b, h = id.h, qblk = id.blk;
  const int q0 = qblk * 256;
  const int myq = q0 + wave * 32 + (lane & 31);
  const int q_lim = (ROWS && a.q_span) ? min(a.q_span[b], a.Tq) : a.Tq;
  if (ROWS && q0 >= q_lim) {
    if (a.dq_colsum && tid < 128) {
      const int nqb128 = (a.Tq + 127) >> 7, blk128 = qblk * 2 + (tid >> 6);
      if (blk128 < nqb128) a.colsum_scratch[((long)(b * nqb128 + blk128) * a.H + h) * 64 + (tid & 63)] = 0.f;
    }
    return;
  }
  const bool w_act = !ROWS || q0 + wave * 32 < q_lim;
  const int myq_c = !w_act ? q0 + (lane & 31) : (myq < a.Tq ? myq : a.Tq - 1);

  bf16x8_t qf[4], dof[4];
  float delta, lse2;
  dq_row_setup<ROWS>(a, b, h, myq, myq_c, w_act, hh, qf, dof, delta, lse2);
  asm volatile("" ::"v"(lse2), "v"(delta), "v"(qf[3]), "v"(dof[3]));
  asm volatile("s_waitcnt vmcnt(0)" ::: "memory");
  bool blk_nz = true;
  if (a.qtile_flags) {
    int* nzs = (int*)smem;
    bool nz = false;
#pragma unroll
    for (int ds = 0; ds < 4; ++ds) {
      const u32x4_t d4 = __builtin_bit_cast(u32x4_t, dof[ds]);
      nz = nz || ((d4[0] | d4[1] | d4[2] | d4[3]) & 0x7fff7fffu) != 0u;
    }
    const bool wnz = __any(nz);
    if (lane == 0) nzs[wave] = wnz ? 1 : 0;
    __syncthreads();
    if (tid < 4) {
      const int ntq = (a.Tq + 63) >> 6, tq = (q0 >> 6) + tid;
      if (tq < ntq) a.qtile_flags[((long)b * a.H + h) * ntq + tq] = nzs[2 * tid] | nzs[2 * tid + 1];
    }
    blk_nz = (nzs[0] | nzs[1] | nzs[2] | nzs[3] | nzs[4] | nzs[5] | nzs[6] | nzs[7]) != 0;
    __syncthreads();
  }

  const int ntiles = (a.Tk + 63) >> 6;
  const int ngroups = (ntiles + PNS - 1) / PNS;
  const PipeSrc1 ksrc = pipe_src1(a.k + (long)b * a.bsk + h * 64, a.ldk, a.Tk, wave, lane);
  const PipeSrc1 vsrc = pipe_src1(a.v + (long)b * a.bsv + h * 64, a.ldv, a.Tk, wave, lane);
  auto dma_tile = [&](int tile, int stage) {
    const unsigned dst = smem_a + stage * PSTG + wave * 1024;
    glds16_asm(ksrc.rs, dst, ksrc.voff + (unsigned)tile * ksrc.tile_bytes);
    glds16_asm(vsrc.rs, dst + TILE, vsrc.voff + (unsigned)tile * vsrc.tile_bytes);
  };

  int ar[4], ac[2][2];
#pragma unroll
  for (int ds = 0; ds < 4; ++ds) ar[ds] = tile_addr(lane & 31, ds * 2 + hh);
  {
    const int G = lane >> 4, i = lane & 15;
    const int row = 4 * (G >> 1) + (i >> 2);
#pragma unroll
    for (int dt = 0; dt < 2; ++dt) {
      const int col = dt * 32 + (G & 1) * 16 + (i & 3) * 4;
      ac[dt][0] = tile_addr(row, col >> 3) + (col & 7) * 2;
      ac[dt][1] = tile_addr(row + 8, col >> 3) + (col & 7) * 2;
    }
  }
  auto rd_rows = [&](int off, int ds) { return *(const bf16x8_t*)(smem + ar[ds] + off); };
  auto rd_tr = [&](int off, int dt, int half) {
    return __builtin_amdgcn_ds_read_tr16_b64_v4i16((lds_s16x4_ptr)(smem + ac[dt][half] + off));
  };

  bf16x8_t Ak[4], Av[4];
  s16x4_t kc[2][2][2];
  f32x16_t dqT[2], S[2], dP[2], ND;
  u32x4_t w[2][2];
#pragma unroll
  for (int i = 0; i < 2; ++i)
#pragma unroll
    for (int r = 0; r < 16; ++r) {
      dqT[i][r] = 0.f;
      S[i][r] = 0.f;
    }
#pragma unroll
  for (int r = 0; r < 16; ++r) ND[r] = -delta;
  dP[0] = ND;
  dP[1] = ND;
  const float c1 = SCALE * LOG2E, nl1 = -lse2;

  auto load_seg = [&](int t, int st, int kt) {
    if (kt == 0) dma_tile(t + 2, (st + 2) & 3);
    const int a_st = kt ? ((st + 1) & 3) : st;
    const int c_st = kt ? st : ((st + 3) & 3);
    const int a_off = a_st * PSTG + (kt ^ 1) * 32 * 128;
    const int c_off = c_st * PSTG + (kt ^ 1) * 32 * 128;
#pragma unroll
    for (int ds = 0; ds < 4; ++ds) {
      Ak[ds] = rd_rows(a_off, ds);
      Av[ds] = rd_rows(a_off + TILE, ds);
    }
#pragma unroll
    for (int u = 0; u < 2; ++u)
#pragma unroll
      for (int dt = 0; dt < 2; ++dt) {
        kc[u][dt][0] = rd_tr(c_off + u * 16 * 128, dt, 0);
        kc[u][dt][1] = rd_tr(c_off + u * 16 * 128, dt, 1);
      }
    if (kt == 0) asm volatile("s_waitcnt vmcnt(2)" ::: "memory");
    asm volatile("s_waitcnt lgkmcnt(0)" ::: "memory");
  };
  auto compute_seg = [&](int kt) {
    const int n = kt ^ 1;
#pragma unroll
    for (int ds = 0; ds < 4; ++ds) {
      if (ds == 0) {
        f32x16_t z;
#pragma unroll
        for (int r = 0; r < 16; ++r) z[r] = 0.f;
        S[n] = MFMA(Ak[0], qf[0], z);
        dP[n] = MFMA(Av[0], dof[0], ND);
      } else {
        S[n] = MFMA(Ak[ds], qf[ds], S[n]);
        dP[n] = MFMA(Av[ds], dof[ds], dP[n]);
      }
      if (ds < 2) {
#pragma unroll
        for (int dt = 0; dt < 2; ++dt) {
          const s16x8_t kv8 = __builtin_shufflevector(kc[ds][dt][0], kc[ds][dt][1], 0, 1, 2, 3, 4, 5, 6, 7);
          dqT[dt] = MFMA(__builtin_bit_cast(bf16x8_t, kv8), __builtin_bit_cast(bf16x8_t, w[n][ds]), dqT[dt]);
        }
      }
    }
#pragma unroll
    for (int j = 0; j < 8; ++j) {
      const float p0 = __builtin_amdgcn_exp2f(fmaf(S[kt][2 * j], c1, nl1));
      const float p1 = __builtin_amdgcn_exp2f(fmaf(S[kt][2 * j + 1], c1, nl1));
      w[kt][j >> 2][j & 3] = pack_bf2(p0 * dP[kt][2 * j], p1 * dP[kt][2 * j + 1]);
    }
#pragma unroll
    for (int i = 0; i < 4; ++i) {
      __builtin_amdgcn_sched_group_barrier(0x008, 1, 0);
      __builtin_amdgcn_sched_group_barrier(0x002, 2, 0);
      __builtin_amdgcn_sched_group_barrier(0x400, 2, 0);
      __builtin_amdgcn_sched_group_barrier(0x002, 2, 0);
      __builtin_amdgcn_sched_group_barrier(0x008, 1, 0);
      __builtin_amdgcn_sched_group_barrier(0x002, 2, 0);
      __builtin_amdgcn_sched_group_barrier(0x400, 1, 0);
      __builtin_amdgcn_sched_group_barrier(0x002, 1, 0);
      __builtin_amdgcn_sched_group_barrier(0x008, 1, 0);
      __builtin_amdgcn_sched_group_barrier(0x002, 2, 0);
      __builtin_amdgcn_sched_group_barrier(0x400, 1, 0);
      __builtin_amdgcn_sched_group_barrier(0x002, 1, 0);
    }
  };

  if (blk_nz) {
  dma_tile(0, 0);
  dma_tile(1, 1);
  asm volatile("s_waitcnt vmcnt(2)" ::: "memory");
  ATTN_BARRIER();
#pragma unroll
  for (int ds = 0; ds < 4; ++ds) {
    Ak[ds] = rd_rows(0, ds);
    Av[ds] = rd_rows(TILE, ds);
  }
#pragma unroll
  for (int ds = 0; ds < 4; ++ds) {
    S[0] = MFMA(Ak[ds], qf[ds], S[0]);
    dP[0] = MFMA(Av[ds], dof[ds], dP[0]);
  }
  ATTN_FENCE();
  load_seg(0, 0, 0);
#pragma unroll
  for (int u = 0; u < 2; ++u) {
    w[1][u] = u32x4_t{0u, 0u, 0u, 0u};
#pragma unroll
    for (int dt = 0; dt < 2; ++dt) {
      kc[u][dt][0] = s16x4_t{0, 0, 0, 0};
      kc[u][dt][1] = s16x4_t{0, 0, 0, 0};
    }
  }
  ATTN_BARRIER();
  if (grp == 1) ATTN_BARRIER();

  for (int g = 0; g < ngroups; ++g) {
#pragma unroll
    for (int st = 0; st < PNS; ++st) {
      const int t = g * PNS + st;
      if (w_act) compute_seg(0);
      ATTN_BARRIER();
      load_seg(t, st, 1);
      ATTN_BARRIER();
      if (w_act) compute_seg(1);
      ATTN_BARRIER();
      load_seg(t + 1, (st + 1) & 3, 0);
      ATTN_BARRIER();
    }
  }
#pragma unroll
  for (int u = 0; u < 2; ++u)
#pragma unroll
    for (int dt = 0; dt < 2; ++dt) {
      const s16x8_t kv8 = __builtin_shufflevector(kc[u][dt][0], kc[u][dt][1], 0, 1, 2, 3, 4, 5, 6, 7);
      dqT[dt] = MFMA(__builtin_bit_cast(bf16x8_t, kv8), __builtin_bit_cast(bf16x8_t, w[1][u]), dqT[dt]);
    }
  if (grp == 0) ATTN_BARRIER();
  asm volatile("s_waitcnt vmcnt(0)" ::: "memory");
  }
  __syncthreads();
  float* wsum = (float*)(smem + 32768);
  {
    const long drow0 = row_at(0L, ROWS, a.q_rows, b, q0 + wave * 32, a.ldq, a.bsq, h);
    store_rows_bf16(smem + wave * 4096, dqT, SCALE, a.dq + drow0, a.ldq, w_act ? a.Tq - (q0 + wave * 32) : 0, lane,
                    a.dq_colsum ? wsum + wave * 64 : nullptr);
  }
  if (a.dq_colsum) {
    __syncthreads();
    if (tid < 128) {
      const int half = tid >> 6, c = tid & 63;
      const int nqb128 = (a.Tq + 127) >> 7;
      const int blk128 = qblk * 2 + half;
      if (blk128 < nqb128)
        a.colsum_scratch[((long)(b * nqb128 + blk128) * a.H + h) * 64 + c] =
            (wsum[half * 256 + c] + wsum[half * 256 + 64 + c]) + (wsum[half * 256 + 128 + c] + wsum[half * 256 + 192 + c]);
    }
  }
}

}

void attn_launch_bwd_dq(const AttnArgs& a, dim3 grid, hipStream_t s) {
  static void (*const kern[2][2])(AttnArgs) = {{attn_bwd_dq_kernel<false, false>, attn_bwd_dq_kernel<false, true>},
                                               {attn_bwd_dq_kernel<true, false>, attn_bwd_dq_kernel<true, true>}};
  hipLaunchKernelGGL(kern[a.causal != 0][a.q_rows != nullptr], grid, dim3(256), 0, s, a);
}

void attn_launch_bwd_dq_pp(const AttnArgs& a, dim3 grid, hipStream_t s) {
  static void (*const kern[2])(AttnArgs) = {attn_bwd_dq_pp_kernel<false>, attn_bwd_dq_pp_kernel<true>};
  hipLaunchKernelGGL(kern[a.q_rows != nullptr], grid, dim3(512), 0, s, a);
}
```

olmoasr_amd/csrc/attention_common.h:

```cpp
#pragma once
#include "decode_shared.h"

namespace {

using dec::LN2;
using dec::LOG2E;
using dec::NEG;
using dec::SCALE;
constexpr int TILE = 64 * 64 * 2;

typedef __attribute__((address_space(3))) s16x4_t* lds_s16x4_ptr;

__device__ __forceinline__ int tile_addr(int row, int c16) {
  const int x = (row >> 1) & 7;
  return row * 128 + ((c16 ^ x ^ ((x & 1) << 2)) << 4);
}

struct TileSrc {
  __amdgpu_buffer_rsrc_t rs;
  unsigned voff[2];
  unsigned row_bytes;
};
__device__ __forceinline__ TileSrc tile_src(const bf16_t* base, long ld, int rmax, int tid) {
  TileSrc t;
  t.rs = __builtin_amdgcn_make_buffer_rsrc(const_cast<bf16_t*>(base), 0, (int)(((long)(rmax - 1) * ld + 64) * 2), 0x00020000);
  t.row_bytes = (unsigned)(ld * 2);
#pragma unroll
  for (int i = 0; i < 2; ++i) {
    const int id = tid + 256 * i;
    t.voff[i] = (unsigned)((id >> 3) * ld * 2 + (id & 7) * 16);
  }
  return t;
}
__device__ __forceinline__ void tile_issue(const TileSrc& t, int row0, u32x4_t (&r)[2]) {
  const unsigned soff = (unsigned)row0 * t.row_bytes;
#pragma unroll
  for (int i = 0; i < 2; ++i) r[i] = __builtin_amdgcn_raw_buffer_load_b128(t.rs, t.voff[i] + soff, 0, 0);
}
__device__ __forceinline__ void tile_commit(char* lds, int tid, const u32x4_t (&r)[2]) {
#pragma unroll
  for (int i = 0; i < 2; ++i) {
    const int id = tid + 256 * i;
    *(u32x4_t*)(lds + tile_addr(id >> 3, id & 7)) = r[i];
  }
}
__device__ __forceinline__ bf16x8_t frag_rows(const char* lds, int sub, int ds, int lane) {
  return *(const bf16x8_t*)(lds + tile_addr(sub + (lane & 31), ds * 2 + (lane >> 5)));
}
__device__ __forceinline__ bf16x8_t frag_cols(const char* lds, int rbase, int csub, int lane) {
  const int G = lane >> 4, i = lane & 15;
  const int row = rbase + 4 * (G >> 1) + (i >> 2);
  const int col = csub + (G & 1) * 16 + (i & 3) * 4;
  const int a0 = tile_addr(row, col >> 3) + (col & 7) * 2;
  const int a1 = tile_addr(row + 8, col >> 3) + (col & 7) * 2;
  const s16x4_t lo = __builtin_amdgcn_ds_read_tr16_b64_v4i16((lds_s16x4_ptr)(lds + a0));
  const s16x4_t hi = __builtin_amdgcn_ds_read_tr16_b64_v4i16((lds_s16x4_ptr)(lds + a1));
  const s16x8_t v = __builtin_shufflevector(lo, hi, 0, 1, 2, 3, 4, 5, 6, 7);
  return __builtin_bit_cast(bf16x8_t, v);
}
__device__ __forceinline__ bf16x8_t pack_half(const f32x16_t& p, int u) {
  u32x4_t o;
#pragma unroll
  for (int i = 0; i < 4; ++i) o[i] = pack_bf2(p[8 * u + 2 * i], p[8 * u + 2 * i + 1]);
  return __builtin_bit_cast(bf16x8_t, o);
}
__device__ __forceinline__ bf16x8_t ld_frag_global(const bf16_t* p) { return __builtin_bit_cast(bf16x8_t, *(const u32x4_t*)p); }
__device__ __forceinline__ int acc_row(int r, int hh) { return (r & 3) + 8 * (r >> 2) + 4 * hh; }
__device__ __forceinline__ void store_rows_bf16(char* stg, const f32x16_t (&T)[2], float scale, bf16_t* gbase, long ld, int rows_valid,
                                                int lane, float* wave_sums = nullptr) {
  const int row = lane & 31, hh = lane >> 5;
#pragma unroll
  for (int dt = 0; dt < 2; ++dt)
#pragma unroll
    for (int g4 = 0; g4 < 4; ++g4) {
      u32x2_t o;
      o[0] = pack_bf2(T[dt][4 * g4] * scale, T[dt][4 * g4 + 1] * scale);
      o[1] = pack_bf2(T[dt][4 * g4 + 2] * scale, T[dt][4 * g4 + 3] * scale);
      *(u32x2_t*)(stg + row * 128 + (((dt * 4 + g4) ^ (row & 7)) << 4) + hh * 8) = o;
    }
  __builtin_amdgcn_wave_barrier();
  float cs[8];
#pragma unroll
  for (int e = 0; e < 8; ++e) cs[e] = 0.f;
#pragma unroll
  for (int i = 0; i < 4; ++i) {
    const int r2 = i * 8 + (lane >> 3), ch = lane & 7;
    const u32x4_t v = *(const u32x4_t*)(stg + r2 * 128 + ((ch ^ (r2 & 7)) << 4));
    if (r2 < rows_valid) {
      *(u32x4_t*)(gbase + (long)r2 * ld + ch * 8) = v;
#pragma unroll
      for (int e = 0; e < 4; ++e) {
        cs[2 * e] += bf_lo(v[e]);
        cs[2 * e + 1] += bf_hi(v[e]);
      }
    }
  }
  if (wave_sums) {
#pragma unroll
    for (int e = 0; e < 8; ++e) {
      float t = cs[e];
      t += __shfl_xor(t, 8, 64);
      t += __shfl_xor(t, 16, 64);
      t += __shfl_xor(t, 32, 64);
      cs[e] = t;
    }
    if (lane < 8) {
#pragma unroll
      for (int e = 0; e < 8; ++e) wave_sums[lane * 8 + e] = cs[e];
    }
  }
  __builtin_amdgcn_wave_barrier();
}

#define MFMA(a, b, c) __builtin_amdgcn_mfma_f32_32x32x16_bf16((a), (b), (c), 0, 0, 0)

__device__ __forceinline__ int chunk_row(const int32_t* rows, int b, int t) { return rows[b * OASR_ROWTAB + (t >> 6)] + (t & 63); }

struct BlockId {
  int b, h, blk;
};
template <bool ROWS>
__device__ __forceinline__ BlockId block_id(const int32_t* tab, int bid, int nblk, int H) {
  BlockId r;
  if (ROWS && tab) {
    const int e = tab[bid];
    r.b = e >> 16;
    r.h = (e >> 4) & 0xfff;
    r.blk = e & 15;
  } else {
    const int bh = bid / nblk;
    r.b = bh / H;
    r.h = bh - r.b * H;
    r.blk = bid - bh * nblk;
  }
  return r;
}

typedef float f32x2_t __attribute__((ext_vector_type(2)));
__device__ __forceinline__ f32x2_t pk_fma(f32x2_t a, f32x2_t b, f32x2_t c) { return __builtin_elementwise_fma(a, b, c); }
__device__ __forceinline__ f32x2_t pk_exp2(f32x2_t a) {
  f32x2_t r;
  r[0] = __builtin_amdgcn_exp2f(a[0]);
  r[1] = __builtin_amdgcn_exp2f(a[1]);
  return r;
}

#define ATTN_FENCE() __builtin_amdgcn_sched_barrier(0)
constexpr int PNS = 4;
constexpr int PSTG = 2 * TILE;

__device__ __forceinline__ void glds16_asm(const u32x4_t rs, unsigned lds_addr, unsigned voff) {
  asm volatile("s_mov_b32 m0, %0\n\ts_nop 0\n\tbuffer_load_dwordx4 %1, %2, 0 offen lds" ::"s"(lds_addr), "v"(voff), "s"(rs) : "memory");
}
struct PipeSrc1 {
  u32x4_t rs;
  unsigned voff;
  unsigned tile_bytes;
};
__device__ __forceinline__ PipeSrc1 pipe_src1(const bf16_t* base, long ld, int rmax, int wave, int lane) {
  PipeSrc1 t;
  const unsigned long addr = (unsigned long)base;
  t.rs[0] = (unsigned)addr;
  t.rs[1] = (unsigned)(addr >> 32) & 0xffffu;
  t.rs[2] = (unsigned)(((long)(rmax - 1) * ld + 64) * 2);
  t.rs[3] = 0x00020000u;
  t.tile_bytes = (unsigned)(64 * ld * 2);
  const int row = wave * 8 + (lane >> 3);
  const int x = (row >> 1) & 7;
  const int c = (lane & 7) ^ x ^ ((x & 1) << 2);
  t.voff = (unsigned)(row * ld * 2 + c * 16);
  return t;
}
#define ATTN_BARRIER()                          \
  do {                                          \
    ATTN_FENCE();                               \
    asm volatile("s_barrier" ::: "memory");     \
    ATTN_FENCE();                               \
  } while (0)

__device__ __forceinline__ int clamped_kv_len(const AttnArgs& a, int b) {
  const int kv_len = a.kv_len ? a.kv_len[b] : a.Tk;
  return kv_len < a.Tk ? kv_len : a.Tk;
}

template <typename P>
__device__ __forceinline__ P row_at(P base, bool chunked, const int32_t* rows, int b, int t, long ld, long bs, int h) {
  return chunked ? base + (long)chunk_row(rows, b, t) * ld + h * 64 : base + (long)b * bs + (long)t * ld + h * 64;
}

template <bool ROWS>
__device__ __forceinline__ void dq_row_setup(const AttnArgs& a, int b, int h, int myq, int myq_c, bool w_act, int hh, bf16x8_t (&qf)[4],
                                             bf16x8_t (&dof)[4], float& delta, float& lse2) {
  const bf16_t* qp = row_at(a.q, ROWS, a.q_rows, b, myq_c, a.ldq, a.bsq, h);
  const long orow_off = row_at(0L, ROWS, a.q_rows, b, myq_c, a.ldo, a.bso, h);
  const bf16_t* dop = a.d_o + orow_off;
  const bf16_t* op = a.o + orow_off;
  const bf16_t* olop = a.o_lo ? a.o_lo + orow_off : nullptr;
  float dpart = 0.f;
#pragma unroll
  for (int ds = 0; ds < 4; ++ds) {
    qf[ds] = ld_frag_global(qp + ds * 16 + hh * 8);
    u32x4_t d4 = *(const u32x4_t*)(dop + ds * 16 + hh * 8);
    if (ROWS && !w_act) d4 = u32x4_t{0u, 0u, 0u, 0u};
    dof[ds] = __builtin_bit_cast(bf16x8_t, d4);
    const u32x4_t o4 = *(const u32x4_t*)(op + ds * 16 + hh * 8);
    if (olop) {
      const u32x4_t r4 = *(const u32x4_t*)(olop + ds * 16 + hh * 8);
#pragma unroll
      for (int i = 0; i < 4; ++i)
        dpart += bf_lo(d4[i]) * (bf_lo(o4[i]) + bf_lo(r4[i])) + bf_hi(d4[i]) * (bf_hi(o4[i]) + bf_hi(r4[i]));
    } else {
#pragma unroll
      for (int i = 0; i < 4; ++i) dpart += bf_lo(d4[i]) * bf_lo(o4[i]) + bf_hi(d4[i]) * bf_hi(o4[i]);
    }
  }
  delta = dpart + __shfl_xor(dpart, 32, 64);
  const long stat_idx = ((long)b * a.H + h) * a.Tq + myq_c;
  if (hh == 0 && myq < a.Tq && w_act) a.delta[stat_idx] = delta;
  lse2 = a.lse[stat_idx] * LOG2E;
}

}

#define ATTN_INTERNAL __attribute__((visibility("hidden")))
ATTN_INTERNAL void attn_launch_fwd(const AttnArgs& a, dim3 grid, hipStream_t s);
ATTN_INTERNAL void attn_launch_decode(const AttnArgs& a, hipStream_t s);
ATTN_INTERNAL void attn_launch_bwd_dq(const AttnArgs& a, dim3 grid, hipStream_t s);
ATTN_INTERNAL void attn_launch_bwd_dq_pp(const AttnArgs& a, dim3 grid, hipStream_t s);
ATTN_INTERNAL void attn_launch_bwd_dkdv(const AttnArgs& a, dim3 grid, hipStream_t s);
ATTN_INTERNAL int attn_launch_bwd_dkdv_pp(const AttnArgs& a, dim3 grid, hipStream_t s);
```

olmoasr_amd/csrc/kernels.h:

```cpp
#pragma once
#include "common.h"
#include "decode_step_core.h"

template <typename T>
struct OperandViewT {
  const T* ptr;
  long ld;
  int rpb;
  long bstride;
  int lead;
  int kvalid;
  int trail_from;
};
typedef OperandViewT<bf16_t> OperandView;
typedef OperandViewT<float> OperandViewF;
template <typename T>
static inline OperandViewT<T> plain_view(const T* p, long ld) {
  return OperandViewT<T>{p, ld, 0, 0, 0, 0, 0};
}

template <typename T>
struct GemmArgsT {
  OperandViewT<T> A, B;
  int M, N, K;
  int ta, tb;
  float alpha;
  const float* bias;
  int act;
  const float* pos;
  int pos_period;
  const T* dgelu_u;
  long ldu;
  const T* resid;
  long ldr;
  T* out;
  T* out_pre;
  long ldc;
  float* out_f32;
  long ldc32;
  float beta;
  float* colsum;
  int atomic;
  int split_k;
  int raster_gm;
  int dgelu_deriv;
  int stagger, stagger_phases;
  int atomic_on_pp;
  int vgrid;
  int epi_flags;
  float* colsum_scratch;
};
typedef GemmArgsT<bf16_t> GemmArgs;
typedef GemmArgsT<float> GemmArgsF;
int launch_gemm(const GemmArgs& a, hipStream_t stream);
int launch_gemm(const GemmArgsF& a, hipStream_t stream);
void gemm_profile_enable(int on);
int gemm_profile_lane(int lane);
void gemm_force_general(int on);
int gemm_set_variant(int v);
void gemm_set_stagger(int sleeps, int phases);
int gemm_profile_collect(double ms[4], double flops[4], long count[4], char* by_symbol, int cap);
int gemm_profile_records(char* buf, int cap);
template <typename T>
static inline GemmArgsT<T> gemm_defaults_t() {
  GemmArgsT<T> g;
  memset(&g, 0, sizeof(g));
  g.alpha = 1.0f;
  g.split_k = 1;
  return g;
}
static inline GemmArgs gemm_defaults() { return gemm_defaults_t<bf16_t>(); }

int launch_layernorm_fwd(const bf16_t* x, const float* gamma, const float* beta, bf16_t* y, float* mean, float* rstd,
                         long rows, int d, hipStream_t s);
int launch_layernorm_bwd(const bf16_t* dy, const bf16_t* x, const float* gamma, const float* mean, const float* rstd,
                         const bf16_t* dres, bf16_t* dx, float* dgamma, float* dbeta, float* dsum, long rows, int d, hipStream_t s);
int launch_layernorm_fwd(const float* x, const float* gamma, const float* beta, float* y, float* mean, float* rstd, long rows, int d,
                         hipStream_t s);
int launch_layernorm_bwd(const float* dy, const float* x, const float* gamma, const float* mean, const float* rstd, const float* dres,
                         float* dx, float* dgamma, float* dbeta, float* dsum, long rows, int d, hipStream_t s);

template <typename T>
struct AttnArgsT {
  const T *q, *k, *v;
  long ldq, ldk, ldv;
  long bsq, bsk, bsv;
  T* o;
  long ldo, bso;
  float* lse;
  T* o_lo;
  const int32_t* kv_len;
  int B, H, Tq, Tk, causal;
  const T* d_o;
  float* delta;
  T *dq, *dk, *dv;
  float *dq_colsum, *dv_colsum;
  float* colsum_scratch;
  int32_t* qtile_flags;
  const int32_t *q_rows, *k_rows;
  const int32_t* q_span;
  const int32_t *qblk128, *qblk256;
  int n128, n256;
};
__host__ __device__ static inline int32_t attn_qblk_pack(int b, int h, int blk) { return (int32_t)((b << 16) | (h << 4) | blk); }
#ifndef OASR_ROWTAB
#define OASR_ROWTAB 16
#endif
static inline size_t attn_colsum_scratch_floats(int B, int H, int Tq, int Tk) {
  return (size_t)B * ((size_t)(Tq + 127) / 128 + (size_t)(Tk + 127) / 128) * H * 64;
}
typedef AttnArgsT<bf16_t> AttnArgs;
typedef AttnArgsT<float> AttnArgsF;
int launch_attention_fwd(const AttnArgs& a, hipStream_t s);
int launch_attention_bwd(const AttnArgs& a, hipStream_t s);
int launch_attention_scores(const AttnArgs& a, float* out, hipStream_t s);
void attention_set_pingpong(int on);
void attention_set_span_grid(int on);
int launch_attention_fwd(const AttnArgsF& a, hipStream_t s);
int launch_attention_bwd(const AttnArgsF& a, hipStream_t s);
int launch_attention_scores(const AttnArgsF& a, float* out, hipStream_t s);

int launch_decode_proj(const bf16_t* x, int M, int K, const bf16_t* W, int N, const float* ln_g, const float* ln_b, const float* bias,
                       int gelu, const bf16_t* resid, long ldr, bf16_t* out, long ldc, float* out_f32, long ldf, hipStream_t s);

struct DecodeStepBufs {
  const bf16_t* wflat;
  const float* params;
  const float* aux;
  bf16_t* cache;
  long cache_lstride;
  bf16_t *x, *x2, *x3, *q, *o, *hg;
  float* part;
  unsigned* ctrl;
};
struct DecodeStepArgs : DecodeStepBufs {
  int d, H, Te, S_max, L, M, pos;
  int flags;
  void* stamps;
  int team, stride;
  const bf16_t* w_logits = nullptr;
  const float *lnf_g = nullptr, *lnf_b = nullptr;
  float* logits_out = nullptr;
  int V = 0;
  DecLayerOffsets l0;
  long lstride, astride;
};
int launch_decode_xcd(const DecodeStepArgs& a, hipStream_t s);
int launch_decode_wide(const DecodeStepArgs& a, hipStream_t s);

int launch_cast_f32_bf16(const float* src, bf16_t* dst, long n, hipStream_t s);
int launch_pack_conv_weight(const float* w, bf16_t* dst, int co, int ci, int ldk, hipStream_t s);
int launch_unpack_conv_grad(const float* g, float* dw, int co, int ci, int ldk, hipStream_t s);
int launch_pack_embedding(const float* e, bf16_t* dst, int rows, int rows_pad, int d, hipStream_t s);
int launch_mel_to_time_major(const float* mel, bf16_t* out, int B, int n_mels, int T, hipStream_t s, const float* clip_max = nullptr);
int launch_embedding_fwd(const int64_t* tok, const float* E, const float* pos, bf16_t* x, int B, int S, int d, long n_embed,
                         hipStream_t s, const int32_t* rows = nullptr);
int launch_embedding_bwd(const int64_t* tok, const bf16_t* dx, float* dE, float* dpos, int B, int S, int d, long pad_id, long n_embed,
                         hipStream_t s, const int32_t* rows = nullptr, const int32_t* span = nullptr);
struct SpanBlockTables {
  int H;
  int32_t *blk128, *blk256;
  int n128, n256;
};
static inline size_t span_block_entries(int B, int S, int H, int gran) { return (size_t)B * ((S + gran - 1) / gran) * H; }
int launch_build_span_tables(const int32_t* span_host, int B, int S, const int64_t* targets, long ignore, int32_t* rows, int32_t* span_dev,
                             int64_t* targets_phys, long* active_rows, hipStream_t s, SpanBlockTables* blocks = nullptr);
int launch_colsum_accum(const bf16_t* x, long ld, long M, int ncols, float* out, hipStream_t s);
int launch_conv2_col2im_dgelu(const bf16_t* dA , const bf16_t* u1 , bf16_t* dpre1, int B, int T1,
                              int d, hipStream_t s);
int launch_conv1_col2im_mel(const bf16_t* dcol, float* dmel, int B, int T1, int n_mels, hipStream_t s);
int launch_conv1_col2im_mel(const float* dcol, float* dmel, int B, int T1, int n_mels, hipStream_t s);
int launch_axpy_f32(const float* src, float* dst, long n, float a, hipStream_t s);
int launch_pack_conv_weight(const float* w, float* dst, int co, int ci, int ldk, hipStream_t s);
int launch_mel_to_time_major(const float* mel, float* out, int B, int n_mels, int T, hipStream_t s, const float* clip_max = nullptr);
int launch_embedding_fwd(const int64_t* tok, const float* E, const float* pos, float* x, int B, int S, int d, long n_embed, hipStream_t s,
                         const int32_t* rows = nullptr);
int launch_embedding_bwd(const int64_t* tok, const float* dx, float* dE, float* dpos, int B, int S, int d, long pad_id, long n_embed,
                         hipStream_t s, const int32_t* rows = nullptr, const int32_t* span = nullptr);
int launch_colsum_accum(const float* x, long ld, long M, int ncols, float* out, hipStream_t s);
int launch_conv2_col2im_dgelu(const float* dA, const float* u1, float* dpre1, int B, int T1, int d, hipStream_t s);
int launch_dgelu_mul(const bf16_t* dy, const bf16_t* u, bf16_t* out, long n, hipStream_t s);
int launch_dgelu_mul(const float* dy, const float* u, float* out, long n, hipStream_t s);
int launch_logits_to_f32(const bf16_t* logits, long ld, long rows, int V, float* out, hipStream_t s);
int launch_logits_to_f32(const float* logits, long ld, long rows, int V, float* out, hipStream_t s);
int launch_dlogits_from_f32(const float* src, int V, long rows, long ld, bf16_t* dst, hipStream_t s);
int launch_dlogits_from_f32(const float* src, int V, long rows, long ld, float* dst, hipStream_t s);

int launch_count_valid(const int64_t* targets, long rows, long ignore, int V, int32_t* n_valid_dev, hipStream_t s);
struct CeReg {
  float eps = 0.f, z = 0.f;
  float* parts = nullptr;
  long parts_stride = 0;
  bool on() const { return eps != 0.f || z != 0.f || parts; }
};
int check_ce_reg(const char* who, float label_smoothing, float z_loss);
int launch_cross_entropy(bf16_t* logits, long ld, int V, const int64_t* targets, long rows, long ignore, float gscale,
                         const int32_t* n_valid_dev, float* row_loss, int write_grad, hipStream_t s, const CeReg& reg = CeReg());
int launch_cross_entropy(float* logits, long ld, int V, const int64_t* targets, long rows, long ignore, float gscale,
                         const int32_t* n_valid_dev, float* row_loss, int write_grad, hipStream_t s, const CeReg& reg = CeReg());
int launch_loss_reduce(const float* row_loss, long rows, const int32_t* n_valid_dev, float mul, float* loss_out, int accumulate,
                       hipStream_t s);

struct SelectArgs {
  const float* logits;
  long ld;
  int V;
  long rows;
  const float *mask, *mask2;
  const int64_t* hist = nullptr;
  long hist_ld = 0;
  int n_hist = -1, ts_begin = 0, eot = 0, no_ts = 0, max_initial_index = -1;
  int64_t* tok = nullptr;
  float* logprob = nullptr;
};
int launch_pick_tokens(const SelectArgs& a, hipStream_t s);
int launch_pick_tokens_ts(const SelectArgs& a, hipStream_t s);
int launch_topk_tokens_ts(const SelectArgs& a, int K, hipStream_t s);
int launch_sample_tokens_ts(const SelectArgs& a, float temperature, const float* u, hipStream_t s);

struct oasr_align_args;
int launch_alignment_matrix(const oasr_align_args* a, void* workspace, size_t workspace_bytes, hipStream_t s);
int launch_dtw(const float* cost, long ld, int N, int M, int negate, int32_t* text_indices, int32_t* time_indices, int32_t* path_len,
               void* workspace, size_t workspace_bytes, hipStream_t s);

struct oasr_edit_args;
int launch_edit_counts(const oasr_edit_args* a, hipStream_t s);

struct oasr_beam_args;
int launch_beam_update(const oasr_beam_args* a, hipStream_t s);
int launch_kv_reorder(void* rows, long layer_stride, int L, int B, int n_ctx, int d, int elem_size, int pos, int group, const int32_t* sources,
                      hipStream_t s);

int launch_argmax_rows(const bf16_t* logits, long ld, int V, long n_rows, const int32_t* rows, const int32_t* span, int B, int S, int32_t* pred,
                       hipStream_t s);
int launch_argmax_rows(const float* logits, long ld, int V, long n_rows, const int32_t* rows, const int32_t* span, int B, int S, int32_t* pred,
                       hipStream_t s);

int launch_score_rows(const bf16_t* logits, long ld, int V, const int64_t* targets, const int32_t* span, int B, int S, long ignore, float* row_nll,
                      int32_t* pred, hipStream_t s);
int launch_score_rows(const float* logits, long ld, int V, const int64_t* targets, const int32_t* span, int B, int S, long ignore, float* row_nll,
                      int32_t* pred, hipStream_t s);
int launch_score_reduce(const float* row_nll, const int32_t* pred, const int64_t* targets, const int32_t* span, int B, int S, int V, long ignore,
                        float* nll_sum, float* nll_max, int32_t* n_tok, int32_t* n_hit, hipStream_t s);

struct oasr_specaug;
int launch_spec_augment(float* mel, int B, int n_mels, int T, const oasr_specaug* policy, uint64_t seed, uint64_t first_clip, hipStream_t s);

struct oasr_speed_args;
int launch_speed_perturb(const oasr_speed_args* a, hipStream_t s);

struct oasr_noise_args;
size_t noise_workspace_bytes(int B, int N);
int launch_noise_mix(const oasr_noise_args* a, hipStream_t s);

struct oasr_reverb_args;
size_t reverb_workspace_bytes(int R, int K);
int launch_reverb(const oasr_reverb_args* a, hipStream_t s);

struct oasr_telephone_args;
int launch_telephone(const oasr_telephone_args* a, hipStream_t s);

int launch_lora_merge(const float* w0, const float* A, const float* B, int rows, int cols, int r, float scale, float* out32, bf16_t* out16,
                      hipStream_t s);
size_t lora_grad_scratch_floats(int rows, int cols, int r);
int launch_lora_grad(const float* dW, const float* A, const float* B, int rows, int cols, int r, float scale, float* dA, float* dB, float* scratch,
                     hipStream_t s);

int launch_grad_stats(const float* g, long n, double* partial , float* stats , hipStream_t s);
int launch_adamw(float* p, const float* g, float* m, float* v, bf16_t* shadow, long n, const float* stats, float inv_scale,
                 float max_norm, float lr, float b1, float b2, float eps, float wd, float bc1, float bc2, hipStream_t s);
int launch_grad_stats_runs(const float* g, const int64_t* runs, int nruns, double* partial , float* stats , hipStream_t s);
int launch_adamw_runs(float* p, const float* g, float* m, float* v, bf16_t* shadow, const int64_t* runs, int nruns, const float* stats,
                      float inv_scale, float max_norm, float lr, float b1, float b2, float eps, float wd, float bc1, float bc2, hipStream_t s);
```

Measured before the change: 6197.

## Make ping-pong attention backward kernels persistent with next-block prefetch overlap

```diff
diff --git a/include/oasr_testing.h b/include/oasr_testing.h
--- a/include/oasr_testing.h
+++ b/include/oasr_testing.h
@@ -16,6 +16,7 @@
 int oasr_xcd_offsets_ok_debug(const int64_t* layer0, long long lstride, long long cache_lstride, int d, int Te, int L, int M);
 int oasr_attention_set_pingpong(int on);
 int oasr_attention_set_span_grid(int on);
+int oasr_attention_set_bwd_persistent(int mode, int grid_cap);
 int oasr_gemm_set_stagger(int sleeps, int phases);
 int oasr_gemm_force_general(int on);
 int oasr_test_gemm(const oasr_gemm_args* a, float* colsum_scratch, int atomic_on_pp, int raster_gm, int stagger, int stagger_phases, void* stream);
diff --git a/olmoasr_amd/_native.py b/olmoasr_amd/_native.py
--- a/olmoasr_amd/_native.py
+++ b/olmoasr_amd/_native.py
@@ -307,6 +307,7 @@
         "oasr_wide_plan_debug": (i32, [i32, i32, i32, i32, i32, i32, vp, i32]),
         "oasr_attention_set_pingpong": (i32, [i32]),
         "oasr_attention_set_span_grid": (i32, [i32]),
+        "oasr_attention_set_bwd_persistent": (i32, [i32, i32]),
         "oasr_profile_gemm_collect": (i32, [vp, vp, vp, C.c_char_p, i32]),
     }
     for name, (res, args) in sig.items():
diff --git a/olmoasr_amd/csrc/api.hip b/olmoasr_amd/csrc/api.hip
--- a/olmoasr_amd/csrc/api.hip
+++ b/olmoasr_amd/csrc/api.hip
@@ -93,6 +93,11 @@
 extern "C" int oasr_attention_set_span_grid(int on) {
   OASR_HOOK_GATE("oasr_attention_set_span_grid");
   attention_set_span_grid(on);
+  return OASR_OK;
+}
+extern "C" int oasr_attention_set_bwd_persistent(int mode, int grid_cap) {
+  OASR_HOOK_GATE("oasr_attention_set_bwd_persistent");
+  attention_set_bwd_persistent(mode, grid_cap);
   return OASR_OK;
 }
 extern "C" int oasr_gemm_force_general(int on) {
diff --git a/olmoasr_amd/csrc/attention.hip b/olmoasr_amd/csrc/attention.hip
--- a/olmoasr_amd/csrc/attention.hip
+++ b/olmoasr_amd/csrc/attention.hip
@@ -4,6 +4,8 @@
 
 int g_attn_pingpong = 1;
 int g_attn_span_grid = 1;
+
+int g_attn_bwd_persistent = 1, g_attn_bwd_grid_cap = 0;
 
 bool span_grid(const AttnArgs& a) { return g_attn_span_grid && a.q_rows && a.q_span && a.qblk128 && a.qblk256; }
 
@@ -29,6 +31,23 @@
 
 void attention_set_pingpong(int on) { g_attn_pingpong = on; }
 void attention_set_span_grid(int on) { g_attn_span_grid = on; }
+void attention_set_bwd_persistent(int mode, int grid_cap) {
+  g_attn_bwd_persistent = mode;
+  g_attn_bwd_grid_cap = grid_cap;
+}
+
+int attn_bwd_persistent_grid(int blocks) {
+  static const int n_cu = [] {
+    int dev = 0, n = 0;
+    if (hipGetDevice(&dev) != hipSuccess || hipDeviceGetAttribute(&n, hipDeviceAttributeMultiprocessorCount, dev) != hipSuccess) n = 256;
+    n &= ~7;
+    return n >= 8 ? n : 8;
+  }();
+  if (!g_attn_bwd_persistent) return blocks;
+  int g = blocks < n_cu ? blocks : n_cu;
+  if (g_attn_bwd_grid_cap > 0 && g_attn_bwd_grid_cap < g) g = g_attn_bwd_grid_cap;
+  return g;
+}
 
 int launch_attention_fwd(const AttnArgs& a, hipStream_t s) {
   int rc = check_args(a, false);
@@ -73,7 +92,8 @@
   }
   const bool pp = !a.causal && !a.kv_len && g_attn_pingpong && (!rows || (!a.k_rows && a.Tq <= 512));
   if (pp) {
-    attn_launch_bwd_dq_pp(aq, gq256, s);
+    rc = attn_launch_bwd_dq_pp(aq, gq256, s);
+    if (rc) return rc;
     rc = attn_launch_bwd_dkdv_pp(a, dim3(cdiv(a.Tk, 256) * a.B * a.H), s);
     if (rc) return rc;
   } else {
diff --git a/olmoasr_amd/csrc/attention_bwd_dkdv.hip b/olmoasr_amd/csrc/attention_bwd_dkdv.hip
--- a/olmoasr_amd/csrc/attention_bwd_dkdv.hip
+++ b/olmoasr_amd/csrc/attention_bwd_dkdv.hip
@@ -196,56 +196,25 @@
 }
 
 constexpr int KSTAT = 2048;
-constexpr int KLDS = KSTAT + PNS * PSTG;
+constexpr int KSTG = KSTAT + PNS * PSTG;
+constexpr int KWS = KSTG + 8 * 4096;
+constexpr int KLDS = KWS + 2048;
 
 __device__ __forceinline__ void glds4_asm(const u32x4_t rs, unsigned lds_addr, unsigned voff) {
   asm volatile("s_mov_b32 m0, %0\n\ts_nop 0\n\tbuffer_load_dword %1, %2, 0 offen lds" ::"s"(lds_addr), "v"(voff), "s"(rs) : "memory");
 }
 
 template <bool ROWS>
-__global__ __launch_bounds__(512, 1) void attn_bwd_dkdv_pp_kernel(AttnArgs a) {
+__global__ __launch_bounds__(512, 1) void attn_bwd_dkdv_pp_kernel(AttnArgs a, int vgrid) {
   extern __shared__ __attribute__((aligned(1024))) char smem[];
   const int tid = threadIdx.x, lane = tid & 63, wave = __builtin_amdgcn_readfirstlane(tid >> 6), hh = lane >> 5;
   const int grp = wave >> 2;
   const unsigned smem_a = (unsigned)(size_t)smem;
   const int nkb = (a.Tk + 255) >> 8;
-  const int bid = xcd_remap(blockIdx.x, gridDim.x);
-  const int bh = bid / nkb;
-  const int b = bh / a.H, h = bh - b * a.H;
-  const int k0 = (bid - bh * nkb) * 256;
-  const int mykey = k0 + wave * 32 + (lane & 31);
-  const int mykey_c = mykey < a.Tk ? mykey : a.Tk - 1;
-
-  const bf16_t* kp = a.k + (long)b * a.bsk + (long)mykey_c * a.ldk + h * 64;
-  const bf16_t* vp = a.v + (long)b * a.bsv + (long)mykey_c * a.ldv + h * 64;
-  bf16x8_t kf[4], vf[4];
-#pragma unroll
-  for (int ds = 0; ds < 4; ++ds) {
-    const u32x4_t k4 = *(const u32x4_t*)(kp + ds * 16 + hh * 8);
-    const u32x4_t v4 = *(const u32x4_t*)(vp + ds * 16 + hh * 8);
-    u32x4_t kn, vn;
-#pragma unroll
-    for (int i = 0; i < 4; ++i) {
-      kn[i] = pack_bf2(bf_lo(k4[i]) * -0.125f, bf_hi(k4[i]) * -0.125f);
-      vn[i] = v4[i] ^ 0x80008000u;
-    }
-    kf[ds] = __builtin_bit_cast(bf16x8_t, kn);
-    vf[ds] = __builtin_bit_cast(bf16x8_t, vn);
-  }
-  asm volatile("" ::"v"(kf[3]), "v"(vf[3]));
-  asm volatile("s_waitcnt vmcnt(0)" ::: "memory");
-
-  int ntiles = (a.Tq + 63) >> 6;
-  if (a.qtile_flags) ntiles = last_nonzero_qtile(a.qtile_flags + ((long)b * a.H + h) * ntiles, ntiles, lane) + 1;
-  if (ROWS && a.q_span) ntiles = min(ntiles, min(a.q_span[b], a.Tq) >> 6);
-  const int ngroups = (ntiles + PNS - 1) / PNS;
-  const PipeSrc1 qsrc = ROWS ? pipe_src1(a.q + h * 64, a.ldq, a.B * a.Tq, wave, lane) : pipe_src1(a.q + (long)b * a.bsq + h * 64, a.ldq, a.Tq, wave, lane);
-  const PipeSrc1 dosrc = ROWS ? pipe_src1(a.d_o + h * 64, a.ldo, a.B * a.Tq, wave, lane) : pipe_src1(a.d_o + (long)b * a.bso + h * 64, a.ldo, a.Tq, wave, lane);
+
+  int b, h, kblk, ntiles, ngroups;
+  PipeSrc1 qsrc, dosrc;
   int qrow[8];
-  if (ROWS) {
-#pragma unroll
-    for (int i = 0; i < 8; ++i) qrow[i] = i < ntiles ? __builtin_amdgcn_readfirstlane(a.q_rows[b * OASR_ROWTAB + i]) : 0x3fffffff;
-  }
   auto qrow_of = [&](int tile) {
     int r = 0x3fffffff;
 #pragma unroll
@@ -253,26 +222,47 @@
     return r;
   };
   u32x4_t srs;
-  {
-    const unsigned long addr = (unsigned long)(((wave & 1) ? a.delta : a.lse) + ((long)b * a.H + h) * a.Tq);
-    srs[0] = (unsigned)addr;
-    srs[1] = (unsigned)(addr >> 32) & 0xffffu;
-    srs[2] = (unsigned)(a.Tq * 4);
-    srs[3] = 0x00020000u;
-  }
   auto dma_tile = [&](int tile, int stage) {
-    const unsigned dst = smem_a + KSTAT + stage * PSTG + wave * 1024;
+    const unsigned dst = __builtin_amdgcn_readfirstlane(smem_a + KSTAT + stage * PSTG + wave * 1024);
+    const unsigned sdst = __builtin_amdgcn_readfirstlane(smem_a + stage * 512 + (wave & 1) * 256);
     if (ROWS) {
       const int r0 = qrow_of(tile);
       const unsigned qo = r0 == 0x3fffffff ? 0x7fffff00u : (unsigned)r0 * (unsigned)(a.ldq * 2);
       const unsigned oo = r0 == 0x3fffffff ? 0x7fffff00u : (unsigned)r0 * (unsigned)(a.ldo * 2);
       glds16_asm(qsrc.rs, dst, r0 == 0x3fffffff ? qo : qsrc.voff + qo);
       glds16_asm(dosrc.rs, dst + TILE, r0 == 0x3fffffff ? oo : dosrc.voff + oo);
-      glds4_asm(srs, smem_a + stage * 512 + (wave & 1) * 256, r0 == 0x3fffffff ? 0x7fffff00u : (unsigned)(lane * 4 + tile * 256));
+      glds4_asm(srs, sdst, r0 == 0x3fffffff ? 0x7fffff00u : (unsigned)(lane * 4 + tile * 256));
     } else {
       glds16_asm(qsrc.rs, dst, qsrc.voff + (unsigned)tile * qsrc.tile_bytes);
       glds16_asm(dosrc.rs, dst + TILE, dosrc.voff + (unsigned)tile * dosrc.tile_bytes);
-      glds4_asm(srs, smem_a + stage * 512 + (wave & 1) * 256, (unsigned)(lane * 4 + tile * 256));
+      glds4_asm(srs, sdst, (unsigned)(lane * 4 + tile * 256));
+    }
+  };
+  auto begin_block = [&](int vb) {
+    const AttnArgs& A = attn_args_reload();
+    const int bid = xcd_remap(vb, vgrid);
+    const int bh = bid / nkb;
+    b = bh / A.H, h = bh - b * A.H;
+    kblk = bid - bh * nkb;
+    ntiles = (A.Tq + 63) >> 6;
+    if (A.qtile_flags) ntiles = last_nonzero_qtile(A.qtile_flags + ((long)b * A.H + h) * ntiles, ntiles, attn_opaque(lane)) + 1;
+    if (ROWS && A.q_span) ntiles = min(ntiles, min(A.q_span[b], A.Tq) >> 6);
+    ngroups = (ntiles + PNS - 1) / PNS;
+    qsrc = ROWS ? pipe_src1(A.q + h * 64, A.ldq, A.B * A.Tq, wave, lane) : pipe_src1(A.q + (long)b * A.bsq + h * 64, A.ldq, A.Tq, wave, lane);
+    dosrc = ROWS ? pipe_src1(A.d_o + h * 64, A.ldo, A.B * A.Tq, wave, lane) : pipe_src1(A.d_o + (long)b * A.bso + h * 64, A.ldo, A.Tq, wave, lane);
+    if (ROWS) {
+#pragma unroll
+      for (int i = 0; i < 8; ++i) qrow[i] = i < ntiles ? __builtin_amdgcn_readfirstlane(A.q_rows[b * OASR_ROWTAB + i]) : 0x3fffffff;
+    }
+    const unsigned long addr = (unsigned long)(((wave & 1) ? A.delta : A.lse) + ((long)b * A.H + h) * A.Tq);
+    srs[0] = (unsigned)addr;
+    srs[1] = (unsigned)(addr >> 32) & 0xffffu;
+    srs[2] = (unsigned)(A.Tq * 4);
+    srs[3] = 0x00020000u;
+    if (ntiles > 0) {
+      dma_tile(0, 0);
+      dma_tile(1, 1);
+      dma_tile(2, 2);
     }
   };
 
@@ -298,13 +288,7 @@
   bf16x8_t Aq[4], Ado[4];
   s16x4_t cq[2][2][2], cdo[2][2][2];
   f32x16_t dkT[2], dvT[2], S[2], dP[2];
-#pragma unroll
-  for (int i = 0; i < 2; ++i)
-#pragma unroll
-    for (int r = 0; r < 16; ++r) {
-      dkT[i][r] = 0.f;
-      dvT[i][r] = 0.f;
-    }
+  bf16x8_t kf[4], vf[4];
 
   auto load_seg = [&](int t, int st, int kt) {
     if (kt == 0) dma_tile(t + 3, (st + 3) & 3);
@@ -377,11 +361,41 @@
     __builtin_amdgcn_sched_group_barrier(0x008, 4, 0);
   };
 
+  begin_block(blockIdx.x);
+  for (int vb = blockIdx.x;;) {
+  const int k0 = kblk * 256;
+  {
+    const AttnArgs& A = attn_args_reload();
+    const int lane_b = attn_opaque(tid) & 63, hh_b = lane_b >> 5;
+    const int mykey = k0 + wave * 32 + (lane_b & 31);
+    const int mykey_c = mykey < A.Tk ? mykey : A.Tk - 1;
+    const bf16_t* kp = A.k + (long)b * A.bsk + (long)mykey_c * A.ldk + h * 64;
+    const bf16_t* vp = A.v + (long)b * A.bsv + (long)mykey_c * A.ldv + h * 64;
+#pragma unroll
+    for (int ds = 0; ds < 4; ++ds) {
+      const u32x4_t k4 = *(const u32x4_t*)(kp + ds * 16 + hh_b * 8);
+      const u32x4_t v4 = *(const u32x4_t*)(vp + ds * 16 + hh_b * 8);
+      u32x4_t kn, vn;
+#pragma unroll
+      for (int i = 0; i < 4; ++i) {
+        kn[i] = pack_bf2(bf_lo(k4[i]) * -0.125f, bf_hi(k4[i]) * -0.125f);
+        vn[i] = v4[i] ^ 0x80008000u;
+      }
+      kf[ds] = __builtin_bit_cast(bf16x8_t, kn);
+      vf[ds] = __builtin_bit_cast(bf16x8_t, vn);
+    }
+    asm volatile("" ::"v"(kf[3]), "v"(vf[3]));
+    asm volatile("s_waitcnt vmcnt(0)" ::: "memory");
+  }
+#pragma unroll
+  for (int i = 0; i < 2; ++i)
+#pragma unroll
+    for (int r = 0; r < 16; ++r) {
+      dkT[i][r] = 0.f;
+      dvT[i][r] = 0.f;
+    }
+
   if (ntiles > 0) {
-  dma_tile(0, 0);
-  dma_tile(1, 1);
-  dma_tile(2, 2);
-  asm volatile("s_waitcnt vmcnt(6)" ::: "memory");
   ATTN_BARRIER();
 #pragma unroll
   for (int ds = 0; ds < 4; ++ds) {
@@ -426,25 +440,33 @@
   asm volatile("s_waitcnt vmcnt(0)" ::: "memory");
   }
   __syncthreads();
+  const int sb = b, sh = h, skblk = kblk;
+  vb += gridDim.x;
+  const bool more = vb < vgrid;
+  if (more) begin_block(vb);
   {
-    char* stg = smem + wave * 4096;
-    const int rows_valid = a.Tk - (k0 + wave * 32);
-    store_rows_bf16(stg, dkT, -SCALE, a.dk + (long)b * a.bsk + (long)(k0 + wave * 32) * a.ldk + h * 64, a.ldk, rows_valid, lane);
-    float* wsum = (float*)(smem + 32768);
-    store_rows_bf16(stg, dvT, 1.0f, a.dv + (long)b * a.bsv + (long)(k0 + wave * 32) * a.ldv + h * 64, a.ldv, rows_valid, lane,
-                    a.dv_colsum ? wsum + wave * 64 : nullptr);
-    if (a.dv_colsum) {
+    const AttnArgs& A = attn_args_reload();
+    const int tid_s = attn_opaque(tid), lane_s = tid_s & 63;
+    char* stg = smem + KSTG + wave * 4096;
+    const int rows_valid = A.Tk - (k0 + wave * 32);
+    store_rows_bf16(stg, dkT, -SCALE, A.dk + (long)sb * A.bsk + (long)(k0 + wave * 32) * A.ldk + sh * 64, A.ldk, rows_valid, lane_s);
+    float* wsum = (float*)(smem + KWS);
+    store_rows_bf16(stg, dvT, 1.0f, A.dv + (long)sb * A.bsv + (long)(k0 + wave * 32) * A.ldv + sh * 64, A.ldv, rows_valid, lane_s,
+                    A.dv_colsum ? wsum + wave * 64 : nullptr);
+    if (A.dv_colsum) {
       __syncthreads();
-      if (tid < 128) {
-        const int half = tid >> 6, c = tid & 63;
-        const int nkb128 = (a.Tk + 127) >> 7;
-        const int blk128 = (bid - bh * nkb) * 2 + half;
-        const long dv_scratch_off = (long)a.B * ((a.Tq + 127) >> 7) * a.H * 64;
+      if (tid_s < 128) {
+        const int half = tid_s >> 6, c = tid_s & 63;
+        const int nkb128 = (A.Tk + 127) >> 7;
+        const int blk128 = skblk * 2 + half;
+        const long dv_scratch_off = (long)A.B * ((A.Tq + 127) >> 7) * A.H * 64;
         if (blk128 < nkb128)
-          a.colsum_scratch[dv_scratch_off + ((long)(b * nkb128 + blk128) * a.H + h) * 64 + c] =
+          A.colsum_scratch[dv_scratch_off + ((long)(sb * nkb128 + blk128) * A.H + sh) * 64 + c] =
               (wsum[half * 256 + c] + wsum[half * 256 + 64 + c]) + (wsum[half * 256 + 128 + c] + wsum[half * 256 + 192 + c]);
       }
     }
+  }
+  if (!more) break;
   }
 }
 
@@ -457,11 +479,12 @@
 }
 
 int attn_launch_bwd_dkdv_pp(const AttnArgs& a, dim3 grid, hipStream_t s) {
-  static void (*const kern[2])(AttnArgs) = {attn_bwd_dkdv_pp_kernel<false>, attn_bwd_dkdv_pp_kernel<true>};
+  static void (*const kern[2])(AttnArgs, int) = {attn_bwd_dkdv_pp_kernel<false>, attn_bwd_dkdv_pp_kernel<true>};
   static LdsAttrOnce attr[2];
   const int rows = a.q_rows != nullptr;
   const int rc = ensure_dynamic_lds(attr[rows], (const void*)kern[rows], KLDS);
   if (rc) return rc;
-  hipLaunchKernelGGL(kern[rows], grid, dim3(512), KLDS, s, a);
+  const int vgrid = (int)grid.x;
+  hipLaunchKernelGGL(kern[rows], dim3(attn_bwd_persistent_grid(vgrid)), dim3(512), KLDS, s, a, vgrid);
   return OASR_OK;
 }
diff --git a/olmoasr_amd/csrc/attention_bwd_dq.hip b/olmoasr_amd/csrc/attention_bwd_dq.hip
--- a/olmoasr_amd/csrc/attention_bwd_dq.hip
+++ b/olmoasr_amd/csrc/attention_bwd_dq.hip
@@ -134,63 +134,41 @@
   }
 }
 
+constexpr int DQ_STG = PNS * PSTG;
+constexpr int DQ_WSUM = DQ_STG + 8 * 4096;
+constexpr int DQ_FLAGS = DQ_WSUM + 2048;
+constexpr int DQ_LDS = DQ_FLAGS + 64;
 template <bool ROWS>
-__global__ __launch_bounds__(512, 1) void attn_bwd_dq_pp_kernel(AttnArgs a) {
-  __shared__ __attribute__((aligned(1024))) char smem[PNS * PSTG];
+__global__ __launch_bounds__(512, 1) void attn_bwd_dq_pp_kernel(AttnArgs a, int vgrid) {
+  extern __shared__ __attribute__((aligned(1024))) char smem[];
   const int tid = threadIdx.x, lane = tid & 63, wave = __builtin_amdgcn_readfirstlane(tid >> 6), hh = lane >> 5;
   const int grp = wave >> 2;
   const unsigned smem_a = (unsigned)(size_t)smem;
   const int nqb = (a.Tq + 255) >> 8;
-  const int bid = xcd_remap(blockIdx.x, gridDim.x);
-  const BlockId id = block_id<ROWS>(a.qblk256, bid, nqb, a.H);
-  const int b = id.b, h = id.h, qblk = id.blk;
-  const int q0 = qblk * 256;
-  const int myq = q0 + wave * 32 + (lane & 31);
-  const int q_lim = (ROWS && a.q_span) ? min(a.q_span[b], a.Tq) : a.Tq;
-  if (ROWS && q0 >= q_lim) {
-    if (a.dq_colsum && tid < 128) {
-      const int nqb128 = (a.Tq + 127) >> 7, blk128 = qblk * 2 + (tid >> 6);
-      if (blk128 < nqb128) a.colsum_scratch[((long)(b * nqb128 + blk128) * a.H + h) * 64 + (tid & 63)] = 0.f;
-    }
-    return;
-  }
-  const bool w_act = !ROWS || q0 + wave * 32 < q_lim;
-  const int myq_c = !w_act ? q0 + (lane & 31) : (myq < a.Tq ? myq : a.Tq - 1);
-
-  bf16x8_t qf[4], dof[4];
-  float delta, lse2;
-  dq_row_setup<ROWS>(a, b, h, myq, myq_c, w_act, hh, qf, dof, delta, lse2);
-  asm volatile("" ::"v"(lse2), "v"(delta), "v"(qf[3]), "v"(dof[3]));
-  asm volatile("s_waitcnt vmcnt(0)" ::: "memory");
-  bool blk_nz = true;
-  if (a.qtile_flags) {
-    int* nzs = (int*)smem;
-    bool nz = false;
-#pragma unroll
-    for (int ds = 0; ds < 4; ++ds) {
-      const u32x4_t d4 = __builtin_bit_cast(u32x4_t, dof[ds]);
-      nz = nz || ((d4[0] | d4[1] | d4[2] | d4[3]) & 0x7fff7fffu) != 0u;
-    }
-    const bool wnz = __any(nz);
-    if (lane == 0) nzs[wave] = wnz ? 1 : 0;
-    __syncthreads();
-    if (tid < 4) {
-      const int ntq = (a.Tq + 63) >> 6, tq = (q0 >> 6) + tid;
-      if (tq < ntq) a.qtile_flags[((long)b * a.H + h) * ntq + tq] = nzs[2 * tid] | nzs[2 * tid + 1];
-    }
-    blk_nz = (nzs[0] | nzs[1] | nzs[2] | nzs[3] | nzs[4] | nzs[5] | nzs[6] | nzs[7]) != 0;
-    __syncthreads();
-  }
-
   const int ntiles = (a.Tk + 63) >> 6;
   const int ngroups = (ntiles + PNS - 1) / PNS;
-  const PipeSrc1 ksrc = pipe_src1(a.k + (long)b * a.bsk + h * 64, a.ldk, a.Tk, wave, lane);
-  const PipeSrc1 vsrc = pipe_src1(a.v + (long)b * a.bsv + h * 64, a.ldv, a.Tk, wave, lane);
+
+  int b, h, qblk, q_lim;
+  bool live;
+  PipeSrc1 ksrc, vsrc;
   auto dma_tile = [&](int tile, int stage) {
     const unsigned dst = smem_a + stage * PSTG + wave * 1024;
     glds16_asm(ksrc.rs, dst, ksrc.voff + (unsigned)tile * ksrc.tile_bytes);
     glds16_asm(vsrc.rs, dst + TILE, vsrc.voff + (unsigned)tile * vsrc.tile_bytes);
   };
+  auto begin_block = [&](int vb) {
+    const AttnArgs& A = attn_args_reload();
+    const BlockId id = block_id<ROWS>(A.qblk256, xcd_remap(vb, vgrid), nqb, A.H);
+    b = id.b, h = id.h, qblk = id.blk;
+    q_lim = (ROWS && A.q_span) ? min(A.q_span[b], A.Tq) : A.Tq;
+    live = !(ROWS && qblk * 256 >= q_lim);
+    ksrc = pipe_src1(A.k + (long)b * A.bsk + h * 64, A.ldk, A.Tk, wave, lane);
+    vsrc = pipe_src1(A.v + (long)b * A.bsv + h * 64, A.ldv, A.Tk, wave, lane);
+    if (live) {
+      dma_tile(0, 0);
+      dma_tile(1, 1);
+    }
+  };
 
   int ar[4], ac[2][2];
 #pragma unroll
@@ -210,22 +188,14 @@
     return __builtin_amdgcn_ds_read_tr16_b64_v4i16((lds_s16x4_ptr)(smem + ac[dt][half] + off));
   };
 
+  bf16x8_t qf[4], dof[4];
   bf16x8_t Ak[4], Av[4];
   s16x4_t kc[2][2][2];
   f32x16_t dqT[2], S[2], dP[2], ND;
   u32x4_t w[2][2];
-#pragma unroll
-  for (int i = 0; i < 2; ++i)
-#pragma unroll
-    for (int r = 0; r < 16; ++r) {
-      dqT[i][r] = 0.f;
-      S[i][r] = 0.f;
-    }
-#pragma unroll
-  for (int r = 0; r < 16; ++r) ND[r] = -delta;
-  dP[0] = ND;
-  dP[1] = ND;
-  const float c1 = SCALE * LOG2E, nl1 = -lse2;
+  const float c1 = SCALE * LOG2E;
+  float nl1;
+  bool w_act;
 
   auto load_seg = [&](int t, int st, int kt) {
     if (kt == 0) dma_tile(t + 2, (st + 2) & 3);
@@ -293,10 +263,52 @@
     }
   };
 
+  int* const nzs = (int*)(smem + DQ_FLAGS);
+  begin_block(blockIdx.x);
+  for (int vb = blockIdx.x;;) {
+  const int q0 = qblk * 256;
+  if (live) {
+  const AttnArgs& A = attn_args_reload();
+  const int tid_b = attn_opaque(tid), lane_b = tid_b & 63;
+  const int myq = q0 + wave * 32 + (lane_b & 31);
+  w_act = !ROWS || q0 + wave * 32 < q_lim;
+  const int myq_c = !w_act ? q0 + (lane_b & 31) : (myq < A.Tq ? myq : A.Tq - 1);
+  float delta, lse2;
+  dq_row_setup<ROWS>(A, b, h, myq, myq_c, w_act, lane_b >> 5, qf, dof, delta, lse2);
+  asm volatile("" ::"v"(lse2), "v"(delta), "v"(qf[3]), "v"(dof[3]));
+  asm volatile("s_waitcnt vmcnt(0)" ::: "memory");
+  bool blk_nz = true;
+  if (A.qtile_flags) {
+    bool nz = false;
+#pragma unroll
+    for (int ds = 0; ds < 4; ++ds) {
+      const u32x4_t d4 = __builtin_bit_cast(u32x4_t, dof[ds]);
+      nz = nz || ((d4[0] | d4[1] | d4[2] | d4[3]) & 0x7fff7fffu) != 0u;
+    }
+    const bool wnz = __any(nz);
+    if (lane_b == 0) nzs[wave] = wnz ? 1 : 0;
+    __syncthreads();
+    if (tid_b < 4) {
+      const int ntq = (A.Tq + 63) >> 6, tq = (q0 >> 6) + tid_b;
+      if (tq < ntq) A.qtile_flags[((long)b * A.H + h) * ntq + tq] = nzs[2 * tid_b] | nzs[2 * tid_b + 1];
+    }
+    blk_nz = (nzs[0] | nzs[1] | nzs[2] | nzs[3] | nzs[4] | nzs[5] | nzs[6] | nzs[7]) != 0;
+    __syncthreads();
+  }
+#pragma unroll
+  for (int i = 0; i < 2; ++i)
+#pragma unroll
+    for (int r = 0; r < 16; ++r) {
+      dqT[i][r] = 0.f;
+      S[i][r] = 0.f;
+    }
+#pragma unroll
+  for (int r = 0; r < 16; ++r) ND[r] = -delta;
+  dP[0] = ND;
+  dP[1] = ND;
+  nl1 = -lse2;
+
   if (blk_nz) {
-  dma_tile(0, 0);
-  dma_tile(1, 1);
-  asm volatile("s_waitcnt vmcnt(2)" ::: "memory");
   ATTN_BARRIER();
 #pragma unroll
   for (int ds = 0; ds < 4; ++ds) {
@@ -346,23 +358,41 @@
   if (grp == 0) ATTN_BARRIER();
   asm volatile("s_waitcnt vmcnt(0)" ::: "memory");
   }
+  } else {
+    const AttnArgs& A = attn_args_reload();
+    if (A.dq_colsum && tid < 128) {
+      const int nqb128 = (A.Tq + 127) >> 7, blk128 = qblk * 2 + (tid >> 6);
+      if (blk128 < nqb128) A.colsum_scratch[((long)(b * nqb128 + blk128) * A.H + h) * 64 + (tid & 63)] = 0.f;
+    }
+  }
   __syncthreads();
-  float* wsum = (float*)(smem + 32768);
-  {
-    const long drow0 = row_at(0L, ROWS, a.q_rows, b, q0 + wave * 32, a.ldq, a.bsq, h);
-    store_rows_bf16(smem + wave * 4096, dqT, SCALE, a.dq + drow0, a.ldq, w_act ? a.Tq - (q0 + wave * 32) : 0, lane,
-                    a.dq_colsum ? wsum + wave * 64 : nullptr);
-  }
-  if (a.dq_colsum) {
-    __syncthreads();
-    if (tid < 128) {
-      const int half = tid >> 6, c = tid & 63;
-      const int nqb128 = (a.Tq + 127) >> 7;
-      const int blk128 = qblk * 2 + half;
-      if (blk128 < nqb128)
-        a.colsum_scratch[((long)(b * nqb128 + blk128) * a.H + h) * 64 + c] =
-            (wsum[half * 256 + c] + wsum[half * 256 + 64 + c]) + (wsum[half * 256 + 128 + c] + wsum[half * 256 + 192 + c]);
-    }
+  const bool s_live = live, s_act = w_act;
+  const int sb = b, sh = h, sqblk = qblk;
+  vb += gridDim.x;
+  const bool more = vb < vgrid;
+  if (more) begin_block(vb);
+  if (s_live) {
+    const AttnArgs& A = attn_args_reload();
+    const int tid_s = attn_opaque(tid);
+    float* wsum = (float*)(smem + DQ_WSUM);
+    {
+      const long drow0 = row_at(0L, ROWS, A.q_rows, sb, q0 + wave * 32, A.ldq, A.bsq, sh);
+      store_rows_bf16(smem + DQ_STG + wave * 4096, dqT, SCALE, A.dq + drow0, A.ldq, s_act ? A.Tq - (q0 + wave * 32) : 0, tid_s & 63,
+                      A.dq_colsum ? wsum + wave * 64 : nullptr);
+    }
+    if (A.dq_colsum) {
+      __syncthreads();
+      if (tid_s < 128) {
+        const int half = tid_s >> 6, c = tid_s & 63;
+        const int nqb128 = (A.Tq + 127) >> 7;
+        const int blk128 = sqblk * 2 + half;
+        if (blk128 < nqb128)
+          A.colsum_scratch[((long)(sb * nqb128 + blk128) * A.H + sh) * 64 + c] =
+              (wsum[half * 256 + c] + wsum[half * 256 + 64 + c]) + (wsum[half * 256 + 128 + c] + wsum[half * 256 + 192 + c]);
+      }
+    }
+  }
+  if (!more) break;
   }
 }
 
@@ -374,7 +404,13 @@
   hipLaunchKernelGGL(kern[a.causal != 0][a.q_rows != nullptr], grid, dim3(256), 0, s, a);
 }
 
-void attn_launch_bwd_dq_pp(const AttnArgs& a, dim3 grid, hipStream_t s) {
-  static void (*const kern[2])(AttnArgs) = {attn_bwd_dq_pp_kernel<false>, attn_bwd_dq_pp_kernel<true>};
-  hipLaunchKernelGGL(kern[a.q_rows != nullptr], grid, dim3(512), 0, s, a);
+int attn_launch_bwd_dq_pp(const AttnArgs& a, dim3 grid, hipStream_t s) {
+  static void (*const kern[2])(AttnArgs, int) = {attn_bwd_dq_pp_kernel<false>, attn_bwd_dq_pp_kernel<true>};
+  static LdsAttrOnce attr[2];
+  const int rows = a.q_rows != nullptr;
+  const int rc = ensure_dynamic_lds(attr[rows], (const void*)kern[rows], DQ_LDS);
+  if (rc) return rc;
+  const int vgrid = (int)grid.x;
+  hipLaunchKernelGGL(kern[rows], dim3(attn_bwd_persistent_grid(vgrid)), dim3(512), DQ_LDS, s, a, vgrid);
+  return OASR_OK;
 }
diff --git a/olmoasr_amd/csrc/attention_common.h b/olmoasr_amd/csrc/attention_common.h
--- a/olmoasr_amd/csrc/attention_common.h
+++ b/olmoasr_amd/csrc/attention_common.h
@@ -178,6 +178,17 @@
     ATTN_FENCE();                               \
   } while (0)
 
+typedef const __attribute__((address_space(4))) AttnArgs* AttnKernArgs;
+__device__ __forceinline__ const AttnArgs& attn_args_reload() {
+  AttnKernArgs p = (AttnKernArgs)__builtin_amdgcn_kernarg_segment_ptr();
+  asm volatile("" : "+s"(p));
+  return *(const AttnArgs*)p;
+}
+__device__ __forceinline__ int attn_opaque(int v) {
+  asm volatile("" : "+v"(v));
+  return v;
+}
+
 __device__ __forceinline__ int clamped_kv_len(const AttnArgs& a, int b) {
   const int kv_len = a.kv_len ? a.kv_len[b] : a.Tk;
   return kv_len < a.Tk ? kv_len : a.Tk;
@@ -226,6 +237,7 @@
 ATTN_INTERNAL void attn_launch_fwd(const AttnArgs& a, dim3 grid, hipStream_t s);
 ATTN_INTERNAL void attn_launch_decode(const AttnArgs& a, hipStream_t s);
 ATTN_INTERNAL void attn_launch_bwd_dq(const AttnArgs& a, dim3 grid, hipStream_t s);
-ATTN_INTERNAL void attn_launch_bwd_dq_pp(const AttnArgs& a, dim3 grid, hipStream_t s);
 ATTN_INTERNAL void attn_launch_bwd_dkdv(const AttnArgs& a, dim3 grid, hipStream_t s);
+ATTN_INTERNAL int attn_launch_bwd_dq_pp(const AttnArgs& a, dim3 grid, hipStream_t s);
 ATTN_INTERNAL int attn_launch_bwd_dkdv_pp(const AttnArgs& a, dim3 grid, hipStream_t s);
+ATTN_INTERNAL int attn_bwd_persistent_grid(int blocks);
diff --git a/olmoasr_amd/csrc/kernels.h b/olmoasr_amd/csrc/kernels.h
--- a/olmoasr_amd/csrc/kernels.h
+++ b/olmoasr_amd/csrc/kernels.h
@@ -116,6 +116,7 @@
 int launch_attention_scores(const AttnArgs& a, float* out, hipStream_t s);
 void attention_set_pingpong(int on);
 void attention_set_span_grid(int on);
+void attention_set_bwd_persistent(int mode, int grid_cap);
 int launch_attention_fwd(const AttnArgsF& a, hipStream_t s);
 int launch_attention_bwd(const AttnArgsF& a, hipStream_t s);
 int launch_attention_scores(const AttnArgsF& a, float* out, hipStream_t s);
```

New measurement: 6212, median of 6. No clear change (+0.2%).
